# microsoft/GenerativeImage2Text

Measured on AMD Instinct MI355X. Metric: captions/sec whole-node (GIT_BASE 224px bs=64/GPU greedy len=20), higher is better.
Workload: dtype f16; 1 GPU; GIT_BASE 224px bs=64/GPU greedy max_len=20 frames=1; global_batch=64, parallelism=dp1, decode_steps_per_caption=19, seq_len_returned=20, hip_graph=True, contexts_in_flight=4, layernorm_folded=True, library=libgitmi_f16.so, encoder_chains=2, schedule=mixed

## Files before the change

generativeimage2text_amd/csrc/engine.hip:

```cpp
#include "../../include/gitmi.h"
#include "engine_state.h"

#include <algorithm>
#include <cmath>
#include <cstdarg>
#include <cstdio>
#include <cstring>

using namespace gitmi;

#ifdef GITMI_EXPERIMENT
#include "../../include/gitmi_experiment.h"
#define GITMI_EXP_EXPORT extern "C"
#else
#define GITMI_EXP_EXPORT [[maybe_unused]] static
#endif

static thread_local char g_err[1024] = "";
int gitmi::fail(const char* fmt, ...) {
    va_list ap;
    va_start(ap, fmt);
    vsnprintf(g_err, sizeof(g_err), fmt, ap);
    va_end(ap);
    return 1;
// ... 224 lines not shown
    hipDeviceSynchronize();
    if (e->enc_after) {
        auto& w = e->enc_after->enc_watchers;
        w.erase(std::remove(w.begin(), w.end(), e), w.end());
    }
    for (gitmi_engine* w : e->enc_watchers) w->enc_after = nullptr;
    destroy_graph(e);
    if (e->own_stream) hipStreamDestroy(e->own_stream);
    if (e->fence_in) hipEventDestroy(e->fence_in);
    if (e->fence_out) hipEventDestroy(e->fence_out);
    for (auto ev : e->gev)
        if (ev) hipEventDestroy(ev);
    if (e->enc_done) hipEventDestroy(e->enc_done);
    for (auto ev : e->event_pool) hipEventDestroy(ev);
    for (void* p : e->allocs) hipFree(p);
    for (void* p : e->sc_allocs) hipFree(p);
    hipFree(e->at_out); hipFree(e->at_stats); hipFree(e->ctx_tab); hipFree(e->mem_tab); hipFree(e->feat_tab); hipFree(e->ban_words);
    if (e->ban_stage) hipHostFree(e->ban_stage);
    if (e->ban_staged) hipEventDestroy(e->ban_staged);
    if (e->trie_off) hipFree(e->trie_off);
    if (e->trie_tok) hipFree(e->trie_tok);
    if (e->trie_child) hipFree(e->trie_child);
    delete e;
}

extern "C" int gitmi_set_image_shape(gitmi_engine* e, int H, int W, void* stream) {
    if (!e) return fail("null engine");
    if (!e->finalized) return fail("weights not finalized");
    const gitmi_config& c = e->cfg;
    if (H == 0 && W == 0) {
        if (!e->ragged) {
            e->ragged = true;
            e->H = e->W = e->gh = e->gw = 0;
            e->N = e->Nmax;
            drop_resident(e);
        }
        return 0;
    }
    if (H < c.patch || W < c.patch) return fail("image %dx%d is smaller than one %d-pixel patch", H, W, c.patch);
    const int gh = H / c.patch, gw = W / c.patch;
    if ((size_t)H * W > e->max_pixels)
        return fail("image %dx%d exceeds the max_image_pixels capacity (%zu)", H, W, e->max_pixels);
    if (gh * gw + 1 > e->Nmax)
        return fail("a %dx%d token grid exceeds the max_image_tokens capacity (%d)", gh, gw, e->Nmax);
    if (H == e->H && W == e->W && !e->ragged) return 0;
    e->ragged = false;
    HIPCK(hipSetDevice(e->device));
    if (gh == e->g_nat && gw == e->g_nat) {
        e->pos_cur = e->w.pos;
    } else {
        HIPCK(launch_pos_bicubic(e->w.pos, e->pos_var, e->g_nat, gh, gw, c.vit_width, (hipStream_t)stream));
        e->pos_cur = e->pos_var;
    }
    e->H = H; e->W = W; e->gh = gh; e->gw = gw; e->N = gh * gw + 1;
    drop_resident(e);
    return 0;
}

static Stream vit_stream(gitmi_engine* e, int M) {
    const int D = e->cfg.vit_width;
    const VitLayerW& L = e->w.vit[0];
    Stream st;
    st.x = e->v_x; st.M = M; st.D = D; st.tag = TAG_GEMM_VIT; st.t = e->v_h;
    st.fold = e->pol.ln_fold && on_p8(e->v_x, D, L.qkv_f.w, e->v_qkv, 3 * D, M, 3 * D, D, false) &&
              on_p8(e->v_x, D, L.ffn1_f.w, e->v_u, 4 * D, M, 4 * D, D, false) && on_p8(e->v_ctx, D, L.wo, e->v_x, D, M, D, D, true) &&
              on_p8(e->v_u, 4 * D, L.w2, e->v_x, D, M, D, 4 * D, true);
    if (st.fold) st.parts[0] = st.parts[1] = e->v_part;
    return st;
}
static Stream prefill_stream(gitmi_engine* e, int M) {
    const int d = e->cfg.dec_hidden, ffn = e->cfg.dec_ffn, D = e->cfg.vit_width;
    const DecLayerW& L = e->w.dec[0];
    Stream st;
    st.x = e->p_y; st.M = M; st.D = d; st.tag = TAG_GEMM_OTHER; st.t = e->p_ht; st.xn = e->p_hf;
    st.fold = e->pol.ln_fold && on_p8(e->feats, D, e->w.vp_w, e->p_y, d, M, d, D, true) &&
              on_p8(e->p_y, d, L.qkv_pf.w, e->img_kv[0], 3 * d, M, 3 * d, d, false) &&
              on_p8(e->p_y, d, L.qkv_pf.w, e->img_kv[0], 3 * d, M, 2 * d, d, false) &&
              (e->cfg.dec_layers < 2 || (on_p8(e->p_y, d, L.ffn1_pf.w, e->p_u, ffn, M, ffn, d, false) &&
                                         on_p8(e->p_ctx, d, L.wo, e->p_y, d, M, d, d, true) && on_p8(e->p_u, ffn, L.w2, e->p_y, d, M, d, ffn, true)));
    if (st.fold) { st.parts[0] = e->p_part[0]; st.parts[1] = e->p_part[1]; }
    return st;
}

static int encode_frames_impl(gitmi_engine* e, const float* const* frames, int F, int B, float* feats_out,
                              hipStream_t s, int stride = 0) {
    const gitmi_config& c = e->cfg;
    const int D = c.vit_width, N = e->N;
    const int F_eff = c.num_frames > 0 ? std::min(F, c.num_frames) : F;
    const int Nimg = stride > 0 ? stride : F_eff * N;
    drop_resident(e);
    SpanGuard phase(e, s, TAG_VIT, 0);
    const int BI = F_eff * B;
    const int M = BI * N;
    const int g2 = N - 1;
    const size_t slot = (size_t)3 * e->max_pixels;
    if (e->ragged)
        HIPCK(launch_im2col_ragged(e->frame_stage[0], slot, e->rg_meta, e->patches, e->pol.f32, B, N, c.patch, e->Kp, e->Kp_pad, s));
    else
    for (int fr = 0; fr < F_eff; ++fr)
        HIPCK(launch_im2col(frames[fr], (char*)e->patches + (size_t)fr * B * g2 * e->Kp_pad * e->pol.esz, e->pol.f32, B,
                            e->H, e->W, c.patch, e->Kp, e->Kp_pad, s));
    RCK(gemm(e, s, e->patches, e->Kp_pad, e->w.conv_w, nullptr, nullptr, 0, e->patch_out, D, true, BI * g2, D, e->Kp_pad, 0,
             TAG_GEMM_VIT));
    Stream x = vit_stream(e, M);
    float2* part = stream_part_out(x);
    if (e->ragged)
        HIPCK(launch_vit_assemble_ragged(e->patch_out, e->w.cls, e->w.pos, e->g_nat, e->rg_meta, e->w.lnpre_g, e->w.lnpre_b, 1e-5f, e->v_x,
                                         e->pol.stream_f16, BI, N, c.patch, D, part, s));
    else
    HIPCK(launch_vit_assemble_ln(e->patch_out, e->w.cls, e->pos_cur, e->w.lnpre_g, e->w.lnpre_b, 1e-5f, e->v_x, e->pol.stream_f16, BI, N, D,
                                 part, D / 256, s));
    stream_written(x, part, e->w.vit[0].ln1g, e->w.vit[0].ln1b, 1e-5f);
    for (int l = 0; l < c.vit_layers; ++l) {
        const VitLayerW& L = e->w.vit[l];
        const VitLayerW* Ln = l + 1 < c.vit_layers ? &e->w.vit[l + 1] : nullptr;
        RCK(ln_gemm(e, s, x, L.qkv_f, L.wqkv, L.bqkv, e->v_qkv, 3 * D, 0, 3 * D, 0));
        RCK(attn_full_packed(e, e->v_qkv, e->v_ctx, D, c.vit_heads, N, BI, e->ragged ? e->rg_ntok : nullptr, s));
        RCK(gemm_to_stream(e, s, x, e->v_ctx, D, L.wo, L.bo, D, true, L.ln2g, L.ln2b, 1e-5f));
        RCK(ln_gemm(e, s, x, L.ffn1_f, L.w1, L.b1, e->v_u, 4 * D, 0, 4 * D, 1));
        RCK(gemm_to_stream(e, s, x, e->v_u, 4 * D, L.w2, L.b2, 4 * D, true, Ln ? Ln->ln1g : nullptr, Ln ? Ln->ln1b : nullptr, 1e-5f));
    }
    for (int fr = 0; fr < F_eff; ++fr) {
        const float* te = (c.num_frames > 0 && e->pol.use_temb) ? e->w.temb[fr] : nullptr;
        if (e->pol.stream_f16) {
            const char* xs = (const char*)e->v_x + (size_t)fr * B * N * D * 2;
            HIPCK(launch_layernorm_s16(xs, D, e->w.lnpost_g, e->w.lnpost_b, 1e-5f, te, e->feats, D, false, nullptr, 0, B * N, D, N,
                                       Nimg, fr * N, s));
            if (feats_out)
                HIPCK(launch_layernorm_s16(xs, D, e->w.lnpost_g, e->w.lnpost_b, 1e-5f, te, feats_out, D, true, nullptr, 0, B * N, D,
                                           N, Nimg, fr * N, s));
        } else {
            HIPCK(launch_layernorm(e->v_x + (size_t)fr * B * N * D, D, e->w.lnpost_g, e->w.lnpost_b, 1e-5f, te, e->feats, D, e->pol.f32,
                                   feats_out, D, B * N, D, N, Nimg, fr * N, s));
        }
    }
    if (e->ragged) {
        HIPCK(launch_zero_pad_rows(e->feats, e->pol.f32, D, e->rg_ntok, B, N, s));
        if (feats_out) HIPCK(launch_zero_pad_rows(feats_out, true, D, e->rg_ntok, B, N, s));
    }

    set_resident(e, B, F_eff, stride);
    return 0;
}

static int kv_repack(gitmi_engine* e, int l, int B, int Nimg, hipStream_t s) {
    const gitmi_config& c = e->cfg;
    void* kh = e->img_kh[l];
    void* vh = e->img_vh[l];
    if (e->pol.f32) HIPCK(launch_kv_repack(e->img_kv[l], kh, vh, B, Nimg, c.dec_heads, c.dec_hidden, s));
    else HIPCK(launch_kv_repack_frag(e->img_kv[l], kh, vh, B, Nimg, round_up(Nimg, 32), c.dec_heads, c.dec_hidden, s));
    return 0;
}

static int prefill_impl(gitmi_engine* e, hipStream_t s) {
    const gitmi_config& c = e->cfg;
    const int d = c.dec_hidden, ffn = c.dec_ffn, D = c.vit_width;
    const int B = e->cur_B, Nimg = e->cur_Nimg, M = B * Nimg;
    e->have_prefill = false;
    SpanGuard phase(e, s, TAG_PREFILL, 0);
    Stream y = prefill_stream(e, M);
    RCK(gemm_to_stream(e, s, y, e->feats, D, e->w.vp_w, e->w.vp_b, D, false, e->w.vp_lng, e->w.vp_lnb, 1e-5f));
    for (int l = 0; l < c.dec_layers; ++l) {
        const DecLayerW& L = e->w.dec[l];
        const bool last = l + 1 == c.dec_layers;
        const int col0 = last ? d : 0;
        RCK(ln_gemm(e, s, y, L.qkv_pf, L.wqkv, L.bqkv, e->img_kv[l], 3 * d, col0, 3 * d - col0, 0));
        RCK(kv_repack(e, l, B, Nimg, s));
        if (last) break;
        RCK(attn_full_packed(e, e->img_kv[l], e->p_ctx, d, c.dec_heads, Nimg, B, key_counts(e), s));
        RCK(gemm_to_stream(e, s, y, e->p_ctx, d, L.wo, L.bo, d, true, L.lnag, L.lnab, 1e-12f));
        RCK(ln_gemm(e, s, y, L.ffn1_pf, L.w1, L.b1, e->p_u, ffn, 0, ffn, 2));
        RCK(gemm_to_stream(e, s, y, e->p_u, ffn, L.w2, L.b2, ffn, true, L.lnog, L.lnob, 1e-12f));
    }
    set_prefilled(e);
    return 0;
}

#ifdef GITMI_EXPERIMENT
#define GITMI_SKIPPED(e, bit) (((e)->pol.decode_skip & (bit)) != 0)
#else
#define GITMI_SKIPPED(e, bit) false
#endif
static int dgemm(gitmi_engine* e, hipStream_t s, const DGemmArgs& g_in) {
    DGemmArgs g = g_in;
    g.dbg = e->pol.dgemm_dbg;
    g.no_row_walk = e->pol.dgemm_no_row_walk >= 0 ? e->pol.dgemm_no_row_walk : e->pol.shared_device ? 0 : 1;
    g.strips_per_wg = e->pol.dgemm_strips >= 0 ? e->pol.dgemm_strips : e->pol.shared_device ? 2 : 1;
    g.rows_per_wg = e->pol.dgemm_rows > 0 ? e->pol.dgemm_rows : g.M > 64 ? 64 : e->pol.shared_device ? 32 : 16;
    SpanGuard sp(e, s, TAG_GEMM_OTHER, gemm_flops(g.M, g.N, g.K));
    HIPCK(launch_dgemm(g, s));
    return 0;
}

static DGemmArgs dgemm_ln(const void* A, const Folded& f, const DLn* ln, void* C, int c_frag, int act, int M, int N, int K) {
    return dgemm_ln(A, f.w, f.bias, f.colsum, ln, C, c_frag, act, M, N, K);
}

static int decode_layers_impl(gitmi_engine* e, const int* kv_src, int ld_ids, int pos, int R, int beams, hipStream_t s) {
    const gitmi_config& c = e->cfg;
    const int d = c.dec_hidden, ffn = c.dec_ffn;
    const int B = R / beams;
    const bool chain = e->pol.skinny && !e->pol.f32;
    for (int l = 0; l < c.dec_layers; ++l) {
        const DecLayerW& L = e->w.dec[l];
        const DecLayerW* Lp = l > 0 ? &e->w.dec[l - 1] : nullptr;
        const DLn ln_prev{e->stats_o, d / 16, 1.0f / (float)d, 1e-12f, Lp ? Lp->lnog : nullptr, Lp ? Lp->lnob : nullptr};
        const DLn ln_a{e->stats_a, d / 16, 1.0f / (float)d, 1e-12f, L.lnag, L.lnab};
        const DLn* ln_o = Lp ? &ln_prev : nullptr;
        AttnDecodeArgs a{};
        a.qkv = e->d_qkv; a.img_k = e->img_kh[l]; a.img_v = e->img_vh[l]; a.txt_k = e->txt_k[l]; a.txt_v = e->txt_v[l]; a.out = e->d_ctx;
        a.kv_src = kv_src; a.ld_src = ld_ids; a.d = d; a.N_img = e->cur_Nimg; a.T_max = c.max_text_len;
        a.img_of = e->img_identity ? nullptr : e->img_of_dev;
        a.pos = pos; a.beams = beams; a.scale = 0.125f;
        a.out_frag = chain ? 1 : 0;
        a.N_pad = round_up(e->cur_Nimg, 32);
        a.dbg = e->pol.attn_dbg;
        a.waves_per_pair = e->pol.attn_nh;
        a.pairs_per_wg = e->pol.attn_pw > 0 ? e->pol.attn_pw : e->pol.shared_device ? 8 : 4;
        const bool stream_ok = !e->pol.shared_device && a.N_pad <= 8 * 32 && B * c.dec_heads >= 384 && e->pol.attn_nh != 2;
        a.stream_wgs = e->pol.attn_stream >= 0 ? e->pol.attn_stream : stream_ok ? 192 : 0;
        if (e->keyed) { a.ntok = e->rg_ntok; a.stream_wgs = 0; }
        bool qkv_inside = false;
        if (chain) {
            const DGemmArgs g = dgemm_ln(l == 0 ? e->d_ht : e->xo_b, L.qkv_f, ln_o, e->d_qkv, 0, 0, R, 3 * d, d);
            attn_decode_set_qkv(a, g);
            qkv_inside = !GITMI_SKIPPED(e, ~0) && !e->pol.dgemm_dbg && attn_decode_qkv_form(a, B, c.dec_heads) && attn_decode_pairs_per_wg(a, B, c.dec_heads) == 8;
            if (!qkv_inside && !GITMI_SKIPPED(e, 2) && !GITMI_SKIPPED(e, 16)) RCK(dgemm(e, s, g));
        } else {
            RCK(gemm(e, s, e->d_ht, d, L.wqkv, L.bqkv, nullptr, 0, e->d_qkv, 3 * d, e->pol.f32, R, 3 * d, d, 0, TAG_GEMM_OTHER));
        }
        if (e->pol.f32) HIPCK(launch_attn_decode(a, B, c.dec_heads, s));
        else if (qkv_inside) HIPCK(launch_attn_decode_qkv(a, B, c.dec_heads, s));
        else if (!GITMI_SKIPPED(e, 1)) HIPCK(launch_attn_decode_mfma(a, B, c.dec_heads, s));
        if (chain) {
            if (!GITMI_SKIPPED(e, 4))
                RCK(dgemm(e, s, dgemm_to_stream(e->d_ctx, L.wo_p, L.bo, l == 0 ? e->d_hf : e->xo_f, ln_o, e->xa_f, e->xa_b, e->stats_a, R, d, d)));
            if (!GITMI_SKIPPED(e, 2)) RCK(dgemm(e, s, dgemm_ln(e->xa_b, L.ffn1_f, &ln_a, e->d_u, 1, 2, R, ffn, d)));
            if (!GITMI_SKIPPED(e, 4))
                RCK(dgemm(e, s, dgemm_to_stream(e->d_u, L.w2_p, L.b2, e->xa_f, &ln_a, e->xo_f, e->xo_b, e->stats_o, R, d, ffn)));
        } else {
            RCK(dec_layer_tail(e, s, L, e->d_ctx, e->d_hf, e->d_ht, e->d_y, e->d_u, R));
        }
    }
    return 0;
}

static int sample_candidates(gitmi_engine* e, const float* logits, int ldl, int R, int step, hipStream_t s, StepCands* cands,
                             const BanArgs* ban);
static int trie_candidates(gitmi_engine* e, const float* logits, int ldl, int cur_len, hipStream_t s, StepCands* cands);
static float rep_penalty_of(const gitmi_engine* e) {
    const double rp = e->sample.repetition_penalty;
    return (e->ss.kind == GITMI_SEARCH_GENERATOR && rp > 0 && rp != 1.0) ? (float)rp : 0.f;
}

static BanArgs ban_args(const gitmi_engine* e) {
    BanArgs b{};
    if (!e->ban_live || !e->ban_words) return b;
    const int mb = e->cfg.max_batch;
    b.W = (e->cfg.vocab + 31) / 32; b.eos = e->cfg.eos;
    const int* tab = reinterpret_cast<const int*>(e->ban_words + (size_t)mb * b.W);
    b.words = e->ban_words; b.set_of = tab; b.min_new = tab + mb; b.ngram = tab + 2 * mb;
    return b;
}

static int decode_head_impl(gitmi_engine* e, const int* ids, int ld_ids, int cur_len, int R, int beams, int suppress_kind,
                            int M, float* logits_out, int ldl, hipStream_t s, StepCands* cands) {
    const gitmi_config& c = e->cfg;
    const int d = c.dec_hidden;
    const bool chain = e->pol.skinny && !e->pol.f32;
    cands->part_val = e->part_val; cands->part_idx = e->part_idx; cands->part_lse = e->part_lse;
    const bool sampling = ids != nullptr && e->ss.sampled;
    const bool trie = ids != nullptr && e->trie_search;
    if ((sampling || trie) && !logits_out) { logits_out = e->logits; ldl = e->ldl; }
    const BanArgs ban = ids ? ban_args(e) : BanArgs{};
    if (chain) {
        VocabArgs v{};
        v.A = (const unsigned short*)e->xo_b; v.lda = d; v.W = (const unsigned short*)e->w.out_f.w; v.bias = e->w.out_f.bias; v.colsum = e->w.out_f.colsum;
        v.stats_in = e->stats_o; v.strips_in = d / 16; v.inv_d = 1.0f / (float)d; v.eps_in = 1e-12f;
        v.M = R; v.N = c.vocab; v.K = d; v.cols_per_wg = e->vocab_cols;
        v.max_wgs = e->pol.vocab_wgs >= 0 ? e->pol.vocab_wgs : (e->pol.shared_device && R <= 64) ? 60 : 0;
        v.ids = ids; v.ld_ids = ld_ids; v.cur_len = cur_len; v.plen = e->plen_dev; v.beams = beams; v.suppress_kind = suppress_kind;
        v.rep_penalty = ids ? rep_penalty_of(e) : 0.f;
        v.ban = ban;
        v.part_val = e->part_val; v.part_idx = e->part_idx; v.part_lse = e->part_lse;
        v.logits_out = logits_out; v.ld_logits = ldl;
        {
            SpanGuard sp(e, s, TAG_GEMM_OTHER, gemm_flops(R, c.vocab, d));
            if (!GITMI_SKIPPED(e, 8)) HIPCK(launch_vocab_topm(v, M, s));
        }
        cands->nparts = e->vocab_nparts; cands->slots = vocab_mtop_slots(M);
        if (sampling) RCK(sample_candidates(e, logits_out, ldl, R, cur_len, s, cands, nullptr));
        if (trie) RCK(trie_candidates(e, logits_out, ldl, cur_len, s, cands));
    } else {
        RCK(gemm(e, s, e->d_ht, d, e->w.out_w, e->w.out_b, nullptr, 0, e->logits, e->ldl, true, R, c.vocab, d, 0, TAG_GEMM_OTHER));
        cands->nparts = 1; cands->slots = row_topm_slots(M);
        if (sampling) RCK(sample_candidates(e, e->logits, e->ldl, R, cur_len, s, cands, &ban));
        else if (trie) RCK(trie_candidates(e, e->logits, e->ldl, cur_len, s, cands));
        else if (ids)
            HIPCK(launch_row_topm(e->logits, e->ldl, c.vocab, ids, ld_ids, cur_len, e->plen_dev, beams, suppress_kind,
                                  rep_penalty_of(e), M, R,
                                  e->part_val, e->part_idx, e->part_lse, s, &ban));
        if (logits_out && logits_out != e->logits) HIPCK(launch_copy_f32(e->logits, e->ldl, logits_out, ldl, R, c.vocab, s));
    }
    return 0;
}

static int check_ready(gitmi_engine* e) {
    if (!e) return fail("null engine");
    if (!e->finalized) return fail("weights not finalized (call gitmi_finalize_weights)");
    HIPCK(hipSetDevice(e->device));
    return 0;
}

static int ragged_prepare(gitmi_engine* e, const float* const* frames, int F, int B, hipStream_t s) {
// ... 69 lines not shown
        RCK(embed_position(e, e->ss.ids[0], T, pos, R, s));
        RCK(decode_layers_impl(e, e->ss.kv_src[0], T, pos, R, beams, s));
        if (pos == t - 1) RCK(decode_head_impl(e, nullptr, T, t, R, beams, 0, 1, logits_out, c.vocab, s, &cands));
    }
    return 0;
}

static int search_begin_impl(gitmi_engine* e, const Request& rq, int V, hipStream_t s) {
    const gitmi_config& c = e->cfg;
    const gitmi_search* sp = rq.sp;
    const int B = rq.Q, minP = rq.minP, maxP = rq.maxP;
    if (!sp) return fail("search: null config");
    if (sp->kind != GITMI_SEARCH_AUTOREGRESSIVE && sp->kind != GITMI_SEARCH_GENERATOR && sp->kind != GITMI_SEARCH_TRIE)
        return fail("search: bad kind");
    if (sp->kind == GITMI_SEARCH_TRIE) {
        if (sp->beam_size != 1) return fail("search: TrieAutoRegressiveBeamSearch asserts beam_size == 1 (trie_decoder.py:37)");
        if (!e->trie_off) return fail("search: no trie loaded (gitmi_set_trie)");
        if (sp->do_sample) return fail("search: the trie search has no sampling branch");
    }
    if (B < 1 || B > c.max_batch) return fail("search: B=%d outside [1,%d]", B, c.max_batch);
    if (sp->beam_size < 1 || sp->beam_size > c.max_beams) return fail("search: beam_size %d outside [1,%d]", sp->beam_size, c.max_beams);
    if (sp->per_node_beam_size < 1 && sp->kind != GITMI_SEARCH_TRIE) return fail("search: per_node_beam_size must be >= 1");
    if (sp->kind == GITMI_SEARCH_GENERATOR && sp->per_node_beam_size < 2)
        return fail("search: GeneratorWithBeamSearch requires per_node_beam_size > 1 (decoder.py:1078)");
    if (sp->beam_size * sp->per_node_beam_size > 16) return fail("search: beam_size*per_node_beam_size > 16 unsupported");
    if (sp->max_steps > c.max_text_len) return fail("search: max_steps %d exceeds max_text_len %d", sp->max_steps, c.max_text_len);
    if (minP < 1 || maxP > sp->max_steps) return fail("search: prefix lengths [%d,%d] outside [1,max_steps]", minP, maxP);
    if (sp->kind == GITMI_SEARCH_GENERATOR && !(sp->length_penalty > 0)) return fail("search: length_penalty must be > 0");
    if (sp->repetition_penalty != 0 && sp->repetition_penalty != 1.0) {
        if (sp->kind != GITMI_SEARCH_GENERATOR) return fail("search: repetition_penalty belongs to GeneratorWithBeamSearch (decoder.py:1064)");
        if (!(sp->repetition_penalty >= 1.0)) return fail("search: `repetition_penalty` should be >= 1 (decoder.py:1080)");
        if (sp->max_steps > 1024) return fail("search: repetition_penalty supports histories up to 1024 tokens");
    }
    if (sp->num_keep_best < 0 || sp->num_keep_best > SS_NHMAX) return fail("search: num_keep_best %d outside [1,%d]", sp->num_keep_best, SS_NHMAX);
    if (sp->num_keep_best > 1 && sp->kind != GITMI_SEARCH_GENERATOR)
        return fail("search: num_keep_best belongs to GeneratorWithBeamSearch.search (decoder.py:1087)");
    if (sp->do_sample) {
        if (sp->kind != GITMI_SEARCH_GENERATOR) return fail("search: do_sample is implemented for GeneratorWithBeamSearch (decoder.py:1146-1166) only");
        if (sp->temperature < 0) return fail("search: temperature must be > 0");
        if (V > 32768) return fail("search: sampling supports vocabularies up to 32768 tokens");
    }
    SearchState& st = e->ss;
    e->trie_search = sp->kind == GITMI_SEARCH_TRIE;
    st.B = B; st.k = sp->beam_size; st.pn = e->trie_search ? 1 : sp->per_node_beam_size;
    st.T = sp->max_steps;
    st.V = V; st.eos = c.eos; st.kind = e->trie_search ? GITMI_SEARCH_AUTOREGRESSIVE : sp->kind; st.length_penalty = sp->length_penalty;
    st.prefixed = rq.prefixed ? 1 : 0;
    st.nh = keep_best(*sp);
    st.sampled = sp->do_sample ? 1 : 0;
    e->sample = *sp;
    st.start = e->start_dev; st.ld_start = c.max_text_len; st.plen = e->plen_dev;
    e->ss_cur = 0; e->ss_len = minP;
    HIPCK(launch_search_init(st, s));
    if (e->trie_search) HIPCK(launch_fill_i32(e->trie_cursor, 0, B, s));
    return 0;
}

static int search_mtop(const SearchState& st) {
    if (st.sampled) return st.pn;
    return st.kind == GITMI_SEARCH_AUTOREGRESSIVE ? std::max(st.k, st.pn) : st.pn * st.k;
}
static int sample_candidates(gitmi_engine* e, const float* logits, int ldl, int R, int step, hipStream_t s, StepCands* cands,
                             const BanArgs* ban) {
    const gitmi_search& sp = e->sample;
    const float temp = sp.temperature > 0 ? (float)sp.temperature : 1.0f;
    HIPCK(launch_sample_rows(logits, ldl, e->ss.V, R, temp, sp.top_k, (float)sp.top_p, e->ss.pn, sp.seed, step,
                             e->part_val, e->part_idx, e->part_lse, nullptr, e->ss.ids[e->ss_cur], e->ss.T, step,
                             rep_penalty_of(e), row_topm_slots(e->ss.pn), s, ban, e->plen_dev, e->ss.k));
    cands->part_val = e->part_val; cands->part_idx = e->part_idx; cands->part_lse = e->part_lse;
    cands->nparts = 1; cands->slots = row_topm_slots(e->ss.pn);
    return 0;
}

static int trie_candidates(gitmi_engine* e, const float* logits, int ldl, int cur_len, hipStream_t s, StepCands* cands) {
    const SearchState& st = e->ss;
    TrieArgs tr{e->trie_off, e->trie_tok, e->trie_child, e->trie_cursor};
    HIPCK(launch_trie_select(logits, ldl, st.V, st.ids[e->ss_cur], st.T, cur_len, e->plen_dev, st.eos, tr, st.B, e->part_val,
                             e->part_idx, e->part_lse, s));
    cands->part_val = e->part_val; cands->part_idx = e->part_idx; cands->part_lse = e->part_lse;
    cands->nparts = 1; cands->slots = 1;
    return 0;
}

static int search_step_impl(gitmi_engine* e, const StepCands& cands, bool embed, hipStream_t s) {
    const SearchState& st = e->ss;
    const int cur_len = e->ss_len;
    if (cur_len >= st.T) return fail("search_advance: sequence already at max_steps");
    HIPCK(launch_search_step(st, e->ss_cur, cur_len, cands, embed_args(e, embed), e->pol.f32, s));
    e->ss_cur ^= 1;
    e->ss_len = cur_len + 1;
    return 0;
}

static int fill_uniform_sentences(gitmi_engine* e, int B, const long long* prefix_dev, int P, hipStream_t s) {
    HIPCK(launch_fill_start(e->start_dev, e->cfg.max_text_len, prefix_dev, 0, 1, e->cfg.sos, B, P, s));
    HIPCK(launch_fill_i32(e->plen_dev, P, B, s));
    e->img_identity = true;
    return 0;
}

extern "C" int gitmi_set_trie(gitmi_engine* e, int n_nodes, const int32_t* child_off, const int32_t* child_tok,
                              const int32_t* child_node) {
    RCK(check_ready(e));
    HIPCK(hipDeviceSynchronize());
    destroy_graph(e);
    int *n_off = nullptr, *n_tok = nullptr, *n_child = nullptr;
    if (n_nodes > 0) {
        if (!child_off || child_off[0] != 0) return fail("set_trie: child_off must start at 0");
        const int n_edges = child_off[n_nodes];
        for (int n = 0; n < n_nodes; ++n)
            if (child_off[n + 1] < child_off[n]) return fail("set_trie: child_off must be non-decreasing");
        if (n_edges > 0 && (!child_tok || !child_node)) return fail("set_trie: null edge arrays");
        for (int i = 0; i < n_edges; ++i)
            if (child_node[i] < 0 || child_node[i] >= n_nodes) return fail("set_trie: edge %d leads to node %d of %d", i, child_node[i], n_nodes);
        hipError_t err = hipMalloc((void**)&n_off, (size_t)(n_nodes + 1) * sizeof(int));
        if (err == hipSuccess) err = hipMalloc((void**)&n_tok, (size_t)std::max(n_edges, 1) * sizeof(int));
        if (err == hipSuccess) err = hipMalloc((void**)&n_child, (size_t)std::max(n_edges, 1) * sizeof(int));
        if (err == hipSuccess) err = hipMemcpy(n_off, child_off, (size_t)(n_nodes + 1) * sizeof(int), hipMemcpyHostToDevice);
        if (err == hipSuccess && n_edges > 0) err = hipMemcpy(n_tok, child_tok, (size_t)n_edges * sizeof(int), hipMemcpyHostToDevice);
        if (err == hipSuccess && n_edges > 0) err = hipMemcpy(n_child, child_node, (size_t)n_edges * sizeof(int), hipMemcpyHostToDevice);
        if (err != hipSuccess) {
            if (n_off) hipFree(n_off);
            if (n_tok) hipFree(n_tok);
            if (n_child) hipFree(n_child);
            return fail("set_trie: %s (the previous trie is kept)", hipGetErrorString(err));
        }
    }
    if (e->trie_off) { hipFree(e->trie_off); hipFree(e->trie_tok); hipFree(e->trie_child); }
    e->trie_off = n_off; e->trie_tok = n_tok; e->trie_child = n_child;
    return 0;
}

static int search_begin_host(gitmi_engine* e, const char* who, const gitmi_search* sp, int B, const int64_t* start_host, int ld,
                             const int32_t* plen_host, int vocab, void* stream) {
    RCK(check_ready(e));
    if (!start_host) return fail("%s: null start", who);
    if (B < 1 || B > e->cfg.max_batch || ld < 1 || ld > e->cfg.max_text_len) return fail("%s: bad B/P", who);
    if (vocab < 2) return fail("%s: bad vocab", who);
    if (sp && sp->kind == GITMI_SEARCH_SCORE) return fail("%s: GITMI_SEARCH_SCORE is not a search (gitmi_generate_prefixed scores sentences)", who);
    if (sp && sp->kind == GITMI_SEARCH_ATTEND) return fail("%s: GITMI_SEARCH_ATTEND is not a search (gitmi_generate_prefixed returns the attention maps of sentences)", who);
    if (sp && sp->kind == GITMI_SEARCH_CONTEXT) return fail("%s: GITMI_SEARCH_CONTEXT is not a search (gitmi_generate_prefixed puts context tokens into the decoder memory)", who);
    if (sp && sp->kind == GITMI_SEARCH_TREE_SCORE) return fail("%s: GITMI_SEARCH_TREE_SCORE is not a search (gitmi_generate_prefixed scores token trees)", who);
    if (sp && sp->kind == GITMI_SEARCH_KEEP) return fail("%s: GITMI_SEARCH_KEEP is not a search (gitmi_generate_prefixed keeps the memory of resident images)", who);
    if (sp && sp->kind == GITMI_SEARCH_RECALL) return fail("%s: GITMI_SEARCH_RECALL is not a search (gitmi_generate_prefixed recalls kept images)", who);
    if (sp && sp->kind == GITMI_SEARCH_FEATURES) return fail("%s: GITMI_SEARCH_FEATURES is not a search (gitmi_generate_prefixed installs given feature rows)", who);
    if (sp && sp->kind == GITMI_SEARCH_CONSTRAIN) return fail("%s: GITMI_SEARCH_CONSTRAIN is not a search (gitmi_generate_prefixed arms the constraints of the next search call)", who);
    if (e->ban_armed)
        return fail("%s: decoding constraints are armed for %d sentences (GITMI_SEARCH_CONSTRAIN): the seam's caller owns its logits and "
                    "applies its own -- disarm first (a GITMI_SEARCH_CONSTRAIN call with Q == 0)", who, e->ban_armed);
    e->ban_live = false;
    int minP = ld, maxP = ld;
    if (plen_host) {
        maxP = 1;
        for (int b = 0; b < B; ++b) {
            if (plen_host[b] < 1 || plen_host[b] > ld) return fail("%s: prefix length %d of sentence %d outside [1,%d]", who, plen_host[b], b, ld);
            minP = std::min(minP, (int)plen_host[b]); maxP = std::max(maxP, (int)plen_host[b]);
        }
    }
    hipStream_t s = (hipStream_t)stream;
    HIPCK(hipMemcpy2DAsync(e->start_dev, (size_t)e->cfg.max_text_len * sizeof(long long), start_host,
                           (size_t)ld * sizeof(long long), (size_t)ld * sizeof(long long), (size_t)B, hipMemcpyHostToDevice, s));
    if (plen_host) HIPCK(hipMemcpyAsync(e->plen_dev, plen_host, (size_t)B * sizeof(int), hipMemcpyHostToDevice, s));
    HIPCK(hipStreamSynchronize(s));
    if (!plen_host) HIPCK(launch_fill_i32(e->plen_dev, ld, B, s));
    e->img_identity = true;
    Request rq{};
    rq.Q = B; rq.minP = minP; rq.maxP = maxP; rq.prefixed = plen_host != nullptr; rq.sp = sp;
    return search_begin_impl(e, rq, vocab, s);
}

extern "C" int gitmi_search_begin(gitmi_engine* e, const gitmi_search* sp, int B, const int64_t* start_host, int P,
// ... 1 lines not shown
    return search_begin_host(e, "search_begin", sp, B, start_host, P, nullptr, vocab, stream);
}

extern "C" int gitmi_search_rows(gitmi_engine* e, int64_t* tokens_out, int* R, int* t, void* stream) {
    RCK(check_ready(e));
    const SearchState& st = e->ss;
    if (R) *R = st.B * st.k;
    if (t) *t = e->ss_len;
    if (tokens_out) HIPCK(launch_search_rows(st, e->ss_cur, e->ss_len, (long long*)tokens_out, (hipStream_t)stream));
    return 0;
}

extern "C" int gitmi_search_advance(gitmi_engine* e, const float* logits, void* stream) {
    RCK(check_ready(e));
    if (!logits) return fail("search_advance: null logits");
    const SearchState& st = e->ss;
    hipStream_t s = (hipStream_t)stream;
    const int M = search_mtop(st), R = st.B * st.k;
    StepCands cands{e->part_val, e->part_idx, e->part_lse, 1, row_topm_slots(M)};
    if (st.sampled) RCK(sample_candidates(e, logits, st.V, R, e->ss_len, s, &cands, nullptr));
    else if (e->trie_search) RCK(trie_candidates(e, logits, st.V, e->ss_len, s, &cands));
    else
        HIPCK(launch_row_topm(logits, st.V, st.V, st.ids[e->ss_cur], st.T, e->ss_len, e->plen_dev, st.k,
                              st.kind == GITMI_SEARCH_AUTOREGRESSIVE ? 1 : 0, rep_penalty_of(e), M, R, e->part_val,
                              e->part_idx, e->part_lse, s));
    return search_step_impl(e, cands, false, s);
}

extern "C" int gitmi_search_done_count(gitmi_engine* e, int* done_out, void* stream) {
    RCK(check_ready(e));
    if (!done_out) return fail("search_done_count: null argument");
    int h = 0;
    HIPCK(hipMemcpyAsync(&h, e->ss.info, sizeof(int), hipMemcpyDeviceToHost, (hipStream_t)stream));
    HIPCK(hipStreamSynchronize((hipStream_t)stream));
    *done_out = h;
    return 0;
}

extern "C" int gitmi_search_finish(gitmi_engine* e, int64_t* tokens_out, float* logprob_out, int32_t* info_out,
                                   void* stream) {
    RCK(check_ready(e));
    const SearchState& st = e->ss;
    HIPCK(launch_search_finish(st, e->ss_cur, e->ss_len, (long long*)tokens_out, logprob_out, info_out, nullptr,
                               (hipStream_t)stream));
    return 0;
}

GITMI_EXP_EXPORT int gitmi_debug_search_begin_prefixed(gitmi_engine* e, const gitmi_search* sp, int B, const int64_t* start_host,
                                                       int ld, const int32_t* plen_host, int vocab, void* stream) {
    if (!plen_host) return fail("debug_search_begin_prefixed: null prefix lengths");
    return search_begin_host(e, "debug_search_begin_prefixed", sp, B, start_host, ld, plen_host, vocab, stream);
}
GITMI_EXP_EXPORT int gitmi_debug_search_advance_lists(gitmi_engine* e, const float* part_val, const int* part_idx,
                                                      const float* part_lse, int nparts, int slots, int embed, void* stream) {
    RCK(check_ready(e));
    if (!part_val || !part_idx || !part_lse) return fail("debug_search_advance_lists: null argument");
    const SearchState& st = e->ss;
    if (st.B < 1 || st.T < 1) return fail("debug_search_advance_lists: no search has begun");
    if (st.sampled || e->trie_search) return fail("debug_search_advance_lists: the sampling and trie searches select from whole logit rows");
    if (nparts < 1 || nparts > 256) return fail("debug_search_advance_lists: nparts=%d outside [1,256]", nparts);
    if (slots != 1 && slots != 2 && slots != 4 && slots != 8 && slots != 16)
        return fail("debug_search_advance_lists: slots=%d is not one of 1, 2, 4, 8, 16", slots);
    if (slots < search_mtop(st)) return fail("debug_search_advance_lists: slots=%d, but the step reads %d candidates per row", slots, search_mtop(st));
    const StepCands cands{part_val, part_idx, (const float2*)part_lse, nparts, slots};
    return search_step_impl(e, cands, embed != 0, (hipStream_t)stream);
}
GITMI_EXP_EXPORT int gitmi_debug_read_hidden(gitmi_engine* e, int R, float* hf_out, void* ht_out, int* ht_frag, int* ht_dtype,
                                             void* stream) {
    RCK(check_ready(e));
    const gitmi_config& c = e->cfg;
    if (R < 1 || R > c.max_batch * c.max_beams) return fail("debug_read_hidden: R=%d outside the capacity", R);
    if (!hf_out || !ht_out || !ht_frag || !ht_dtype) return fail("debug_read_hidden: null argument");
    hipStream_t s = (hipStream_t)stream;
    const size_t D = (size_t)c.dec_hidden, Rp = (size_t)(R + 15) / 16 * 16;
    HIPCK(hipMemcpyAsync(hf_out, e->d_hf, (size_t)R * D * sizeof(float), hipMemcpyDefault, s));
    HIPCK(hipMemcpyAsync(ht_out, e->d_ht, Rp * D * e->pol.esz, hipMemcpyDefault, s));
    HIPCK(hipStreamSynchronize(s));
    *ht_frag = (e->pol.skinny && !e->pol.f32) ? 1 : 0;
    *ht_dtype = e->pol.f32 ? GITMI_DTYPE_F32 : gitmi_operand_dtype();
    return 0;
}

static int generate_encode(gitmi_engine* e, const Request& rq, hipStream_t s) {
    RCK(encode_frames_impl(e, rq.frames, rq.F, rq.B, nullptr, s));
    return prefill_impl(e, s);
}
static int images_ready(gitmi_engine* e, const Request& rq, hipStream_t s) {
    if (rq.frames) return generate_encode(e, rq, s);
    return e->have_prefill ? 0 : prefill_impl(e, s);
}

static int generate_decode(gitmi_engine* e, const Request& rq, hipStream_t s, bool allow_poll) {
    const gitmi_config& c = e->cfg;
    const gitmi_search* sp = rq.sp;
    RCK(search_begin_impl(e, rq, c.vocab, s));
    const int Q = rq.Q, minP = rq.minP, maxP = rq.maxP, T = sp->max_steps, k = sp->beam_size, R = Q * k;
    const SearchState& st = e->ss;
    const int M = search_mtop(st);
    const int suppress = sp->kind != GITMI_SEARCH_GENERATOR ? 1 : 0;
    {
        SpanGuard phase(e, s, TAG_DECODE, 0);
        RCK(embed_position(e, st.ids[0], T, 0, R, s));
        e->ss_len = 1;
        StepCands cands{e->part_val, e->part_idx, e->part_lse, 1, 1};
        while (e->ss_len < T) {
            const int cur_len = e->ss_len;
            SpanGuard step(e, s, TAG_STEP, 0);
            RCK(decode_layers_impl(e, st.kv_src[e->ss_cur], T, cur_len - 1, R, k, s));
            if (cur_len >= minP)
                RCK(decode_head_impl(e, st.ids[e->ss_cur], T, cur_len, R, k, suppress, M, nullptr, 0, s, &cands));
            RCK(search_step_impl(e, cands, true, s));
            if (allow_poll && e->ss_len > maxP && (e->ss_len - maxP) % 8 == 0 && e->ss_len < T) {
                int h[4];
                HIPCK(hipMemcpyAsync(h, st.info, sizeof(h), hipMemcpyDeviceToHost, s));
                HIPCK(hipStreamSynchronize(s));
                if (h[0] >= Q) break;
            }
        }
    }
    HIPCK(launch_search_finish(st, e->ss_cur, e->ss_len, rq.tokens, rq.logprob, rq.info, rq.sent, s));
    if (e->ragged)
        HIPCK(launch_ragged_report(e->rg_meta, e->img_identity ? nullptr : e->img_of_dev, Q, keep_best(*sp), rq.logprob, rq.info,
                                   nullptr, s));
    const double kv = (double)Q * c.dec_layers * 2.0 * ((double)e->cur_Nimg + k * 0.5 * (minP + T)) * c.dec_hidden * e->pol.esz;
    e->last_decode_step_bytes = e->w.dec_weight_bytes + kv;
    return 0;
}

static int generate_body(gitmi_engine* e, const Request& rq, hipStream_t s, bool allow_poll) {
    SpanGuard total(e, s, 99, 0);
    RCK(images_ready(e, rq, s));
    return generate_decode(e, rq, s, allow_poll);
}

static GraphKey graph_key_of(const gitmi_engine* e, const Request& rq, int F_eff) {
    const gitmi_search& sp = *rq.sp;
    const bool resident = rq.frames == nullptr;
    return {rq.B, rq.Q, F_eff, rq.minP, sp.kind, sp.beam_size, sp.per_node_beam_size, sp.max_steps, e->H, e->W,
            rq.prefixed ? 1 : 0, e->img_identity ? 1 : 0, e->pol.use_temb ? 1 : 0, resident ? 1 : 0,
            resident ? e->cur_Nimg : 0, resident && e->keyed ? 1 : 0, sp.length_penalty,
            sp.do_sample, sp.top_k, keep_best(sp), sp.top_p, sp.temperature, sp.repetition_penalty, sp.seed, e->ban_live ? 1 : 0};
}

static int replay(gitmi_engine* e, const Request& rq, hipStream_t x, const CapturedGraph* enc, const CapturedGraph* dec) {
    const bool timed = e->profile_mode == 2;
    if (timed) {
        for (auto& ev : e->gev)
            if (!ev) HIPCK(hipEventCreate(&ev));
        HIPCK(hipEventRecord(e->gev[enc ? 0 : 1], x));
    } else if (enc && e->enc_after && e->enc_after->enc_done) {
        HIPCK(hipStreamWaitEvent(x, e->enc_after->enc_done, 0));
    }
    if (enc) {
        HIPCK(enc->launch(x));
        if (timed) HIPCK(hipEventRecord(e->gev[1], x));
        else if (e->enc_done && !e->enc_watchers.empty()) HIPCK(hipEventRecord(e->enc_done, x));
    }
    if (dec) HIPCK(dec->launch(x));
    if (!timed) return 0;
    HIPCK(hipEventRecord(e->gev[2], x));
    HIPCK(hipStreamSynchronize(x));
    float a = 0, b = 0;
    if (enc) HIPCK(hipEventElapsedTime(&a, e->gev[0], e->gev[1]));
    HIPCK(hipEventElapsedTime(&b, e->gev[1], e->gev[2]));
    e->split_encode_ms += a; e->split_decode_ms += b; e->split_calls += 1; e->split_steps += rq.sp->max_steps - 1;
    return 0;
}

static int generate_graphed(gitmi_engine* e, const Request& rq, hipStream_t s) {
    const gitmi_config& c = e->cfg;
    const bool resident = rq.frames == nullptr;
    hipStream_t x = s ? s : e->own_stream;
    if (x != s) {
        HIPCK(hipEventRecord(e->fence_in, s));
        HIPCK(hipStreamWaitEvent(x, e->fence_in, 0));
    }
    const size_t frame_bytes = (size_t)rq.B * 3 * e->H * e->W * sizeof(float);
    const int F_eff = resident ? e->cur_F : c.num_frames > 0 ? std::min(rq.F, c.num_frames) : rq.F;
    if (!e->ragged && !resident)
    for (int f = 0; f < F_eff; ++f)
        HIPCK(hipMemcpyAsync(e->frame_stage[f], rq.frames[f], frame_bytes, hipMemcpyDeviceToDevice, x));
    Request own = rq;
    if (!resident) { own.frames = e->frame_stage.data(); own.F = F_eff; }
    own.tokens = e->out_tokens; own.logprob = e->out_lp; own.info = e->out_info; own.sent = e->out_sent;
    const GraphKey key = graph_key_of(e, rq, F_eff);
    const CapturedGraph *enc = nullptr, *dec = nullptr;
    if (resident) {
        RCK(images_ready(e, rq, x));
        if (!e->follow_slot.valid || !(key == e->follow_slot.key)) {
            e->follow_slot.valid = false;
            RCK(e->graph_follow.capture(x, [&] { return generate_decode(e, own, x, false); }));
            e->follow_slot = {key, true};
        }
        dec = &e->graph_follow;
    } else {
        const bool split = e->profile_mode == 2 || e->enc_after != nullptr || !e->enc_watchers.empty();
        if (!e->full_slot.valid || !(key == e->full_slot.key) || split != e->graph_is_split) {
            e->full_slot.valid = false;
            e->graph_decode.reset();
            if (!split) {
                RCK(e->graph_full.capture(x, [&] { return generate_body(e, own, x, false); }));
            } else {
                RCK(e->graph_full.capture(x, [&] { return generate_encode(e, own, x); }));
                RCK(e->graph_decode.capture(x, [&] { return generate_decode(e, own, x, false); }));
            }
            e->full_slot = {key, true}; e->graph_is_split = split;
        } else {
            set_resident(e, rq.B, F_eff);
            set_prefilled(e);
        }
        enc = &e->graph_full;
        if (split) dec = &e->graph_decode;
    }
    RCK(replay(e, rq, x, enc, dec));
    const size_t nout = (size_t)rq.Q * (size_t)keep_best(*rq.sp);
    HIPCK(hipMemcpyAsync(rq.tokens, e->out_tokens, nout * rq.sp->max_steps * sizeof(long long), hipMemcpyDefault, x));
    HIPCK(hipMemcpyAsync(rq.logprob, e->out_lp, nout * sizeof(float), hipMemcpyDefault, x));
    HIPCK(hipMemcpyAsync(rq.info, e->out_info, 4 * sizeof(int), hipMemcpyDefault, x));
    if (rq.sent != e->out_sent) HIPCK(hipMemcpyAsync(rq.sent, e->out_sent, (size_t)rq.Q * 2 * sizeof(int), hipMemcpyDefault, x));
    if (x != s) {
        HIPCK(hipEventRecord(e->fence_out, x));
        HIPCK(hipStreamWaitEvent(s, e->fence_out, 0));
    }
    return 0;
}

static int generate_run(gitmi_engine* e, const Request& rq, hipStream_t s, bool constrained) {
    const bool long_budget = rq.sp->max_steps - rq.minP > 32;
    const bool graph = e->pol.use_graph && !e->profiling && !long_budget;
    if (constrained) e->ban_armed = 0;
    e->ban_live = constrained;
    const int rc = settle_residency(e, rq, graph ? generate_graphed(e, rq, s) : generate_body(e, rq, s, long_budget && !e->profiling));
    e->ban_live = false;
    return rc;
}

static int constrain_check(const gitmi_engine* e, const char* who, const gitmi_search* sp, int Q, bool* constrained);

extern "C" int gitmi_generate(gitmi_engine* e, const float* const* frames, int F, int B, const int64_t* prefix, int P,
                              const gitmi_search* sp, int64_t* tokens_out, float* logprob_out, int32_t* info_out,
                              void* stream) {
    RCK(check_ready(e));
    const gitmi_config& c = e->cfg;
    if (sp && sp->kind == GITMI_SEARCH_SCORE) return fail("generate: GITMI_SEARCH_SCORE scores given sentences: call gitmi_generate_prefixed");
    if (sp && sp->kind == GITMI_SEARCH_ATTEND) return fail("generate: GITMI_SEARCH_ATTEND maps given sentences: call gitmi_generate_prefixed");
    if (sp && sp->kind == GITMI_SEARCH_CONTEXT) return fail("generate: GITMI_SEARCH_CONTEXT takes context segments: call gitmi_generate_prefixed");
    if (sp && sp->kind == GITMI_SEARCH_TREE_SCORE) return fail("generate: GITMI_SEARCH_TREE_SCORE scores given token trees: call gitmi_generate_prefixed");
    if (sp && sp->kind == GITMI_SEARCH_KEEP) return fail("generate: GITMI_SEARCH_KEEP keeps the memory of resident images: call gitmi_generate_prefixed");
    if (sp && sp->kind == GITMI_SEARCH_RECALL) return fail("generate: GITMI_SEARCH_RECALL recalls kept images: call gitmi_generate_prefixed");
    if (sp && sp->kind == GITMI_SEARCH_FEATURES) return fail("generate: GITMI_SEARCH_FEATURES installs given feature rows: call gitmi_generate_prefixed");
    if (sp && sp->kind == GITMI_SEARCH_CONSTRAIN) return fail("generate: GITMI_SEARCH_CONSTRAIN arms decoding constraints: call gitmi_generate_prefixed");
    if (!frames) RCK(check_resident(e, "generate", B));
    if (!sp || !tokens_out || !logprob_out || !info_out) return fail("generate: null argument");
    if (frames) RCK(check_frames(e, "generate", frames, F, B));
    if (!prefix) P = 1;
    if (P < 1 || P > c.max_text_len) return fail("generate: prefix length %d outside [1,%d]", P, c.max_text_len);
    if (sp->max_steps < P || sp->max_steps > c.max_text_len) return fail("generate: max_steps %d outside [P,%d]", sp->max_steps, c.max_text_len);
    bool constrained = false;
    RCK(constrain_check(e, "generate", sp, B, &constrained));
    hipStream_t s = (hipStream_t)stream;
    if (frames) RCK(ragged_prepare(e, frames, F, B, s));
    RCK(fill_uniform_sentences(e, B, (const long long*)prefix, P, s));
    const Request rq{frames, F, B, B, P, P, false, sp, (long long*)tokens_out, logprob_out, info_out, e->out_sent};
    return generate_run(e, rq, s, constrained);
}

static int tree_max_depth(const gitmi_config& c) { return std::min((int)c.max_text_len, (int)c.max_pos); }
constexpr int TREE_MAX_ROWS = 65535 * 64;
static void score_free(gitmi_engine* e) {
    for (void* p : e->sc_allocs) hipFree(p);
    e->sc_allocs.clear();
    e->sc_rows = 0;
    e->tr_out_n = 0;
}
static int score_alloc(gitmi_engine* e, size_t rows_needed, size_t tree_out = 0) {
    size_t rows = (size_t)round_up((int)rows_needed, 128);
    if (e->sc_rows >= rows && e->tr_out_n >= tree_out) return 0;
    rows = std::max(rows, e->sc_rows);
    tree_out = std::max(tree_out, e->tr_out_n);
    score_free(e);
    const gitmi_config& c = e->cfg;
    const int d = c.dec_hidden;
    const size_t Qmax = (size_t)c.max_batch * c.max_beams;
    const size_t esz = e->pol.esz;
    auto alloc = [&](auto** p, size_t bytes) -> bool {
        void* q = nullptr;
        if (hipMalloc(&q, bytes) != hipSuccess) return false;
        e->sc_allocs.push_back(q);
        *reinterpret_cast<void**>(p) = q;
        return true;
    };
    const bool ok = alloc(&e->sc_hf, rows * d * 4) && alloc(&e->sc_y, rows * d * 4) && alloc(&e->sc_ht, rows * d * esz) &&
                    alloc(&e->sc_qkv, rows * 3 * d * esz) && alloc(&e->sc_ctx, rows * d * esz) &&
                    alloc(&e->sc_u, rows * c.dec_ffn * esz) &&
                    alloc(&e->sc_part, rows * (size_t)(e->pol.f32 ? 1 : score_head_tiles(c.vocab)) * sizeof(float4)) &&
                    alloc(&e->sc_zt, rows * 4) && alloc(&e->sc_tgt, rows * 4) && alloc(&e->sc_lens, Qmax * 4) &&
                    alloc(&e->sc_img, Qmax * 4) && alloc(&e->sc_bad, Qmax * 4) && alloc(&e->sc_info, 16) &&
// ... 722 lines not shown
```

generativeimage2text_amd/csrc/engine_state.h:

```cpp
#pragma once
#include "../../include/gitmi.h"
#include "abi_common.h"
#include "launchers.h"

#include <hip/hip_runtime.h>

#include <functional>
#include <map>
#include <string>
#include <tuple>
#include <vector>

static inline int round_up(int x, int m) { return (x + m - 1) / m * m; }
static inline int keep_best(const gitmi_search& sp) { return sp.num_keep_best > 1 ? sp.num_keep_best : 1; }

struct HostTensor {
    std::vector<float> data;
    std::vector<int64_t> shape;
    float amax = 0.f;
    size_t numel() const { size_t n = 1; for (auto s : shape) n *= (size_t)s; return n; }
};

struct Folded { void* w = nullptr; float* bias = nullptr; float* colsum = nullptr; };

struct VitLayerW {
    void *wqkv = nullptr, *wo = nullptr, *w1 = nullptr, *w2 = nullptr;
    float *bqkv = nullptr, *bo = nullptr, *b1 = nullptr, *b2 = nullptr;
    float *ln1g = nullptr, *ln1b = nullptr, *ln2g = nullptr, *ln2b = nullptr;
    Folded qkv_f;
    Folded ffn1_f;
};
struct DecLayerW {
    void *wqkv = nullptr, *wo = nullptr, *w1 = nullptr, *w2 = nullptr;
    float *bqkv = nullptr, *bo = nullptr, *b1 = nullptr, *b2 = nullptr;
    float *lnag = nullptr, *lnab = nullptr, *lnog = nullptr, *lnob = nullptr;
    Folded qkv_f;
    Folded ffn1_f;
    void *wo_p = nullptr, *w2_p = nullptr;
    Folded qkv_pf, ffn1_pf;
};

struct TimedSpan { hipEvent_t a, b; int tag; double flops; };
enum { TAG_VIT = 0, TAG_PREFILL = 1, TAG_DECODE = 2, TAG_GEMM_VIT = 10, TAG_GEMM_OTHER = 11, TAG_STEP = 20 };

struct GraphKey {
    int B, Q, F, P, kind, k, pn, T, H, W, prefixed, ident, temb, resident, Nimg, keyed; double lp;
    int smp, top_k, nh; double top_p, temp, rp; unsigned long long seed;
    int constrained;
    auto fields() const {
        return std::tie(B, Q, F, P, kind, k, pn, T, H, W, prefixed, ident, temb, resident, Nimg, keyed, lp, smp, top_k, nh, top_p, temp,
                        rp, seed, constrained);
    }
    bool operator==(const GraphKey& o) const { return fields() == o.fields(); }
};
struct GraphSlot { GraphKey key{}; bool valid = false; };

struct CapturedGraph {
    hipGraph_t graph = nullptr;
    hipGraphExec_t exec = nullptr;
    void reset() {
        if (exec) hipGraphExecDestroy(exec);
        if (graph) hipGraphDestroy(graph);
        exec = nullptr, graph = nullptr;
    }
    int capture(hipStream_t s, const std::function<int()>& fn);
    hipError_t launch(hipStream_t s) const { return hipGraphLaunch(exec, s); }
};

struct Request {
    const float* const* frames;
    int F, B, Q, minP, maxP;
    bool prefixed;
    const gitmi_search* sp;
    long long* tokens; float* logprob; int32_t* info;
    int32_t* sent;
};

struct ModelWeights {
    void* conv_w = nullptr;
    float *cls = nullptr, *pos = nullptr, *lnpre_g = nullptr, *lnpre_b = nullptr, *lnpost_g = nullptr, *lnpost_b = nullptr;
    std::vector<VitLayerW> vit;
    std::vector<float*> temb;
    void* vp_w = nullptr;
    float *vp_b = nullptr, *vp_lng = nullptr, *vp_lnb = nullptr;
    float *words_f = nullptr, *positions_f = nullptr, *emb_lng = nullptr, *emb_lnb = nullptr;
    std::vector<DecLayerW> dec;
    void* out_w = nullptr;
    float* out_b = nullptr;
    Folded out_f;
    double dec_weight_bytes = 0;
};

struct Policy {
    bool f32 = false;
    size_t esz = 2;
    int attn_impl = 1;
    bool stream_f16 = false;
    bool ln_fold = false;
    bool ln_fold_ready = false;
    bool skinny = true;
    bool use_graph = true;
    bool use_temb = true;
    bool shared_device = false;
    int attn_dbg = 0, dgemm_dbg = 0;
    int attn_pw = 0;
    int attn_nh = 0;
    int attn_stream = -1;
    int dgemm_no_row_walk = -1;
    int dgemm_strips = -1;
    int vocab_wgs = -1;
    int gemm_tall = 1;
    int dgemm_rows = 0;
    int decode_skip = 0;
};

struct gitmi_engine {
    gitmi_config cfg{};
    ModelWeights w;
    Policy pol;
    int device = 0;
    bool finalized = false;
    gitmi_engine* parent = nullptr;

    std::map<std::string, HostTensor> host_w;
    std::vector<void*> allocs;

    int N = 0, gh = 0, gw = 0, H = 0, W = 0, Kp = 0, Kp_pad = 0;
    int N_nat = 0, g_nat = 0, Nmax = 0;
    size_t max_pixels = 0;
    float* pos_var = nullptr;
    const float* pos_cur = nullptr;
    bool ragged = false;
    int4* rg_meta = nullptr;
    int* rg_ntok = nullptr;
    bool keyed = false;
    bool has_context = false;
    int* ctx_tab = nullptr;
    size_t ctx_tab_ints = 0;
    gitmi::MemoryEntry* mem_tab = nullptr;
    size_t mem_tab_n = 0;
    std::vector<int4> res_desc;
    gitmi::FeaturePiece* feat_tab = nullptr;
    unsigned int* ban_words = nullptr;
    int* ban_stage = nullptr;
    hipEvent_t ban_staged = nullptr;
    int ban_armed = 0;
    bool ban_live = false;

    void *patches = nullptr, *v_h = nullptr, *v_qkv = nullptr, *v_ctx = nullptr, *v_u = nullptr;
    float *patch_out = nullptr, *v_x = nullptr;
    void* feats = nullptr;
    float *p_y = nullptr, *p_hf = nullptr;
    void *p_ht = nullptr, *p_ctx = nullptr, *p_u = nullptr;
    std::vector<void*> img_kv;
    std::vector<void*> img_kh, img_vh;
    float *d_y = nullptr, *d_hf = nullptr, *logits = nullptr;
    void *d_ht = nullptr, *d_qkv = nullptr, *d_ctx = nullptr, *d_u = nullptr;
    std::vector<void*> txt_k, txt_v;
// ... 63 lines not shown
```

generativeimage2text_amd/csrc/engine_weights.hip:

```cpp
#include "engine_state.h"

#include <algorithm>
#include <cmath>
#include <cstring>

using namespace gitmi;

static int dev_alloc(gitmi_engine* e, void** p, size_t bytes) {
    if (bytes == 0) bytes = 16;
    HIPCK(hipMalloc(p, bytes));
    e->allocs.push_back(*p);
    return 0;
}
template <typename T> static int dev_alloc_t(gitmi_engine* e, T** p, size_t count) {
    return dev_alloc(e, reinterpret_cast<void**>(p), count * sizeof(T));
}

static float half_to_float(uint16_t h) {
    const uint32_t sign = (uint32_t)(h & 0x8000) << 16;
    uint32_t exp = (h >> 10) & 0x1f, man = h & 0x3ff, out;
    if (exp == 0) {
        if (man == 0) out = sign;
        else {
            exp = 127 - 15 + 1;
// ... 103 lines not shown
    RCK(dev_alloc(e, &e->patches, (size_t)c.max_batch * c.max_frames * (e->Nmax - 1) * e->Kp_pad * esz));
    RCK(dev_alloc_t(e, &e->patch_out, (size_t)c.max_batch * c.max_frames * (e->Nmax - 1) * D));
    RCK(dev_alloc_t(e, &e->pos_var, (size_t)e->Nmax * D));
    RCK(dev_alloc_t(e, &e->v_x, Mv * D));
    RCK(dev_alloc(e, &e->v_h, Mv * D * esz));
    RCK(dev_alloc(e, &e->v_qkv, Mv * 3 * D * esz));
    RCK(dev_alloc(e, &e->v_ctx, Mv * D * esz));
    RCK(dev_alloc(e, &e->v_u, Mv * 4 * D * esz));
    RCK(dev_alloc(e, &e->feats, Mp * D * esz));
    if (e->pol.ln_fold_ready) {
        RCK(dev_alloc_t(e, &e->v_part, Mv * 4));
        RCK(dev_alloc_t(e, &e->p_part[0], Mp * 4));
        RCK(dev_alloc_t(e, &e->p_part[1], Mp * 4));
        HIPCK(hipMemset(e->v_part, 0, Mv * 4 * sizeof(float2)));
        HIPCK(hipMemset(e->p_part[0], 0, Mp * 4 * sizeof(float2)));
        HIPCK(hipMemset(e->p_part[1], 0, Mp * 4 * sizeof(float2)));
    }
    RCK(dev_alloc_t(e, &e->p_y, Mp * d));
    RCK(dev_alloc_t(e, &e->p_hf, Mp * d));
    RCK(dev_alloc(e, &e->p_ht, Mp * d * esz));
    RCK(dev_alloc(e, &e->p_ctx, Mp * d * esz));
    RCK(dev_alloc(e, &e->p_u, Mp * c.dec_ffn * esz));
    e->img_kv.resize(c.dec_layers);
    e->img_kh.resize(c.dec_layers);
    e->img_vh.resize(c.dec_layers);
    e->txt_k.resize(c.dec_layers);
    e->txt_v.resize(c.dec_layers);
    for (int l = 0; l < c.dec_layers; ++l) {
        RCK(dev_alloc(e, &e->img_kv[l], Mp * 3 * d * esz));
        const size_t Mkv = (size_t)c.max_batch * round_up(c.max_frames * e->Nmax, 32);
        RCK(dev_alloc(e, &e->img_kh[l], Mkv * d * esz));
        RCK(dev_alloc(e, &e->img_vh[l], Mkv * d * esz));
        RCK(dev_alloc(e, &e->txt_k[l], R * T * d * esz));
        RCK(dev_alloc(e, &e->txt_v[l], R * T * d * esz));
    }
    RCK(dev_alloc_t(e, &e->d_y, R * d));
    RCK(dev_alloc_t(e, &e->d_hf, R * d));
    RCK(dev_alloc(e, &e->d_ht, R * d * esz));
    RCK(dev_alloc(e, &e->d_qkv, R * 3 * d * esz));
    RCK(dev_alloc(e, &e->d_ctx, R * d * esz));
    RCK(dev_alloc(e, &e->d_u, R * c.dec_ffn * esz));
    RCK(dev_alloc_t(e, &e->xa_f, R * d));
    RCK(dev_alloc_t(e, &e->xo_f, R * d));
    RCK(dev_alloc(e, &e->xa_b, R * d * 2));
    RCK(dev_alloc(e, &e->xo_b, R * d * 2));
    RCK(dev_alloc_t(e, &e->stats_a, R * (size_t)(d / 16)));
    RCK(dev_alloc_t(e, &e->stats_o, R * (size_t)(d / 16)));
    e->ldl = round_up(c.vocab, 8);
    RCK(dev_alloc_t(e, &e->logits, R * e->ldl));
    e->vocab_cols = 128;
    e->vocab_nparts = (e->pol.skinny && !e->pol.f32) ? vocab_parts(c.vocab, e->vocab_cols) : 1;
    RCK(dev_alloc_t(e, &e->part_val, R * (size_t)e->vocab_nparts * 16));
    RCK(dev_alloc_t(e, &e->part_idx, R * (size_t)e->vocab_nparts * 16));
    RCK(dev_alloc_t(e, &e->part_lse, R * (size_t)e->vocab_nparts));
    SearchState& s = e->ss;
    for (int i = 0; i < 2; ++i) {
        RCK(dev_alloc_t(e, &s.ids[i], R * T));
        RCK(dev_alloc_t(e, &s.kv_src[i], R * T));
        RCK(dev_alloc_t(e, &s.score[i], R));
    }
    RCK(dev_alloc_t(e, &s.done, (size_t)c.max_batch));
    RCK(dev_alloc_t(e, &s.hyp_n, (size_t)c.max_batch));
    RCK(dev_alloc_t(e, &s.hyp_cnt, (size_t)c.max_batch));
    RCK(dev_alloc_t(e, &s.hyp_worst, (size_t)c.max_batch));
    RCK(dev_alloc_t(e, &s.hyp_score, (size_t)c.max_batch * SS_NHMAX));
    RCK(dev_alloc_t(e, &s.hyp_len, (size_t)c.max_batch * SS_NHMAX));
    RCK(dev_alloc_t(e, &s.hyp_seq, (size_t)c.max_batch * SS_NHMAX));
    RCK(dev_alloc_t(e, &s.hyp_tok, (size_t)c.max_batch * SS_NHMAX * T));
    RCK(dev_alloc_t(e, &s.stop, (size_t)c.max_batch));
    RCK(dev_alloc_t(e, &s.early, (size_t)c.max_batch));
    RCK(dev_alloc_t(e, &s.info, 4));
    RCK(dev_alloc_t(e, &s.len_norm, (size_t)T + 1));
    RCK(dev_alloc_t(e, &e->start_dev, (size_t)c.max_batch * T));
    RCK(dev_alloc_t(e, &e->plen_dev, (size_t)c.max_batch));
    RCK(dev_alloc_t(e, &e->img_of_dev, (size_t)c.max_batch));
    RCK(dev_alloc_t(e, &e->trie_cursor, (size_t)c.max_batch));
    RCK(dev_alloc_t(e, &e->out_tokens, (size_t)c.max_batch * SS_NHMAX * T));
    RCK(dev_alloc_t(e, &e->out_lp, (size_t)c.max_batch * SS_NHMAX));
    RCK(dev_alloc_t(e, &e->out_info, 4));
    RCK(dev_alloc_t(e, &e->out_sent, (size_t)c.max_batch * 2));
    HIPCK(hipStreamCreateWithFlags(&e->own_stream, hipStreamNonBlocking));
    HIPCK(hipEventCreateWithFlags(&e->fence_in, hipEventDisableTiming));
    HIPCK(hipEventCreateWithFlags(&e->fence_out, hipEventDisableTiming));
    e->frame_stage.resize(c.max_frames);
    for (int f = 0; f < c.max_frames; ++f)
        RCK(dev_alloc_t(e, &e->frame_stage[f], (size_t)c.max_batch * 3 * e->max_pixels));
    RCK(dev_alloc_t(e, &e->rg_meta, (size_t)c.max_batch));
    RCK(dev_alloc_t(e, &e->rg_ntok, (size_t)c.max_batch));
    return 0;
}

#ifdef GITMI_OPS_F16
static inline float bf16_round(float f) { return (float)(_Float16)f; }
#else
static inline float bf16_round(float f) {
    uint32_t u;
    memcpy(&u, &f, 4);
    if ((u & 0x7f800000u) == 0x7f800000u) return f;
    u += 0x7fffu + ((u >> 16) & 1u);
    u &= 0xffff0000u;
    memcpy(&f, &u, 4);
    return f;
}
#endif
static int fold_layernorm(gitmi_engine* e, const std::vector<float>& W, const std::vector<float>& bias,
                          const std::vector<float>& gamma, const std::vector<float>& beta, int64_t rows, int K, bool frag,
                          Folded* out) {
    std::vector<float> wf((size_t)rows * K), b2((size_t)rows), c2((size_t)rows);
    float amax = 0.f;
    for (int64_t n = 0; n < rows; ++n) {
        double sum = 0.0, cst = bias[n];
        const float* w = &W[(size_t)n * K];
        float* o = &wf[(size_t)n * K];
        for (int k = 0; k < K; ++k) {
            amax = std::max(amax, std::fabs(w[k] * gamma[k]));
            o[k] = bf16_round(w[k] * gamma[k]);
            sum += (double)o[k];
            cst += (double)beta[k] * (double)w[k];
        }
        c2[n] = (float)sum;
        b2[n] = (float)cst;
    }
    RCK(operand_range_check(e, "a matrix with the LayerNorm gain in front of it folded in (W . gamma)", amax));
    const int64_t rows_pad = (rows + 127) / 128 * 128;
    RCK(dev_alloc(e, &out->w, (size_t)rows_pad * K * 2));
    float* tmp = nullptr;
    void* tmp_b = nullptr;
    HIPCK(hipMalloc((void**)&tmp, wf.size() * 4));
    hipError_t err = hipSuccess;
    if (frag) err = hipMalloc(&tmp_b, wf.size() * 2);
    if (err == hipSuccess) err = hipMemcpy(tmp, wf.data(), wf.size() * 4, hipMemcpyHostToDevice);
    if (err == hipSuccess) err = launch_convert_pad(tmp, frag ? tmp_b : out->w, false, (size_t)rows, K, K, 0);
    if (err == hipSuccess && frag) err = launch_frag_pack(tmp_b, out->w, (int)rows, (int)rows_pad, K, 0);
    if (err == hipSuccess) err = hipDeviceSynchronize();
    hipFree(tmp);
    if (tmp_b) hipFree(tmp_b);
    HIPCK(err);
    b2.resize((size_t)rows_pad, 0.f);
    c2.resize((size_t)rows_pad, 0.f);
    RCK(dev_alloc_t(e, &out->bias, (size_t)rows_pad));
    RCK(dev_alloc_t(e, &out->colsum, (size_t)rows_pad));
    HIPCK(hipMemcpy(out->bias, b2.data(), (size_t)rows_pad * 4, hipMemcpyHostToDevice));
    HIPCK(hipMemcpy(out->colsum, c2.data(), (size_t)rows_pad * 4, hipMemcpyHostToDevice));
    return 0;
}
static int pack_frag(gitmi_engine* e, const void* src, int64_t rows, int K, void** dst) {
    const int64_t rows_pad = (rows + 15) / 16 * 16;
    RCK(dev_alloc(e, dst, (size_t)rows_pad * K * 2));
    HIPCK(launch_frag_pack(src, *dst, (int)rows, (int)rows_pad, K, 0));
    HIPCK(hipDeviceSynchronize());
    return 0;
}
static int fold_named(gitmi_engine* e, const std::string& ln, const std::string& dense, int64_t rows, int K, bool frag, Folded* out) {
    const HostTensor *g, *b, *w, *bi;
    RCK(get_w(e, ln + "weight", {K}, &g));
    RCK(get_w(e, ln + "bias", {K}, &b));
    RCK(get_w(e, dense + "weight", {rows, K}, &w));
    RCK(get_w(e, dense + "bias", {rows}, &bi));
    return fold_layernorm(e, w->data, bi->data, g->data, b->data, rows, K, frag, out);
}
static std::string vit_layer_key(int i) { return "image_encoder.transformer.resblocks." + std::to_string(i) + "."; }
static std::string dec_layer_key(int i) { return "textual.transformer.encoder.layer." + std::to_string(i) + "."; }
static int concat_qkv(gitmi_engine* e, const std::string& pre, int d) {
    HostTensor w, b;
    w.shape = {3 * d, d};
    b.shape = {3 * d};
    for (const char* name : {"query", "key", "value"}) {
        const HostTensor *tw, *tb;
        RCK(get_w(e, pre + "attention.self." + name + ".weight", {d, d}, &tw));
// ... 151 lines not shown
```

generativeimage2text_amd/csrc/kernels_attn_decode.hip:

```cpp
#include "gitmi_common.h"
#include "launchers.h"
#include "dgemm_shared.h"
#include <algorithm>
#include <type_traits>

#pragma clang fp contract(off)

namespace gitmi {

static constexpr int HD = 64;

__global__ __launch_bounds__(256) void kv_repack_frag_kernel(const bf16_t* __restrict__ qkv, bf16_t* __restrict__ kf,
                                                             bf16_t* __restrict__ vt, int N, int Np, int H, int d) {
    __shared__ bf16_t vs[32][HD + 8];
    const int s = blockIdx.x, h = blockIdx.y, b = blockIdx.z, tid = threadIdx.x;
    const int nsteps = Np >> 5;
    bf16_t* kdst = kf + ((size_t)b * H + h) * Np * HD;
    bf16_t* vdst = vt + ((size_t)b * H + h) * Np * HD;
    const int key = tid >> 3, ch = tid & 7;
    const int n = s * 32 + key;
    u32x4_t kv = {0u, 0u, 0u, 0u}, vv = kv;
    if (n < N) {
        const bf16_t* src = qkv + ((size_t)b * N + n) * 3 * d + d + h * HD + ch * 8;
        kv = *reinterpret_cast<const u32x4_t*>(src);
        vv = *reinterpret_cast<const u32x4_t*>(src + d);
    }
    *reinterpret_cast<u32x4_t*>(kdst + frag_tile(n >> 4, ch >> 2, 2, (ch & 3) * 16 + (n & 15))) = kv;
    *reinterpret_cast<u32x4_t*>(&vs[key][ch * 8]) = vv;
    __syncthreads();
    const int dt = tid >> 6, lane = tid & 63, lg = lane >> 4, dim = dt * 16 + (lane & 15);
    bf16_t o[8];
#pragma unroll
    for (int e = 0; e < 8; ++e) o[e] = vs[(e >> 2) * 16 + lg * 4 + (e & 3)][dim];
    u32x4_t ov;
#pragma unroll
    for (int e = 0; e < 4; ++e) ov[e] = (uint32_t)o[2 * e] | ((uint32_t)o[2 * e + 1] << 16);
    *reinterpret_cast<u32x4_t*>(vdst + (((size_t)s * 4 + dt) * 64 + lane) * 8) = ov;
}

__device__ __forceinline__ void unpack8(const u32x4_t& r, float (&v)[8]) {
#pragma unroll
    for (int i = 0; i < 4; ++i) {
        unpack2op(r[i], v[2 * i], v[2 * i + 1]);
    }
}
__device__ __forceinline__ void ld8bf(const bf16_t* p, float (&v)[8]) { unpack8(*reinterpret_cast<const u32x4_t*>(p), v); }

constexpr int ACS = 4;

struct Pair {
    int h, row0;
    bool on;
};

struct QkvSrc {
    const bf16_t* q0;
    int row_stride, part;
    __device__ __forceinline__ const bf16_t* q(int j) const { return q0 + (size_t)j * row_stride; }
    __device__ __forceinline__ const bf16_t* k(int j) const { return q(j) + part; }
    __device__ __forceinline__ const bf16_t* v(int j) const { return q(j) + 2 * part; }
};
__device__ __forceinline__ QkvSrc qkv_rows(const AttnDecodeArgs& a, const Pair& p) {
    return QkvSrc{reinterpret_cast<const bf16_t*>(a.qkv) + (size_t)p.row0 * (3 * a.d) + p.h * HD, 3 * a.d, a.d};
}

template <int KB>
__device__ __forceinline__ void load_text_kv(const AttnDecodeArgs& a, const Pair& p, const QkvSrc& qs, int j, int s, int sub, u32x4_t& kr, u32x4_t& vr) {
    if (s == a.pos) {
        kr = *reinterpret_cast<const u32x4_t*>(qs.k(j) + sub * 8);
        vr = *reinterpret_cast<const u32x4_t*>(qs.v(j) + sub * 8);
    } else {
        const int srow = KB == 1 ? p.row0 : a.kv_src[(size_t)(p.row0 + j) * a.ld_src + s];
        const size_t off = ((size_t)srow * a.T_max + s) * a.d + p.h * HD + sub * 8;
        kr = *reinterpret_cast<const u32x4_t*>(reinterpret_cast<const bf16_t*>(a.txt_k) + off);
        vr = *reinterpret_cast<const u32x4_t*>(reinterpret_cast<const bf16_t*>(a.txt_v) + off);
    }
}

template <int KB, int TI>
struct TextItems {
    int j[TI];
    u32x4_t kr[TI], vr[TI];
    __device__ __forceinline__ void load(const AttnDecodeArgs& a, const Pair& p, const QkvSrc& qs, int grp, int ngrp, int sub) {
        const int nt = a.pos + 1;
#pragma unroll
// ... 242 lines not shown
    auto load_chunk = [&](int s0) {
#pragma unroll
        for (int c = 0; c < ACS; ++c) {
            const int s = s0 + NH * c;
            const bool on = s < nimg_steps && !(a.dbg & 8);
            const bf16_t* kp = Kf + frag_tile(2 * s, 0, 2, lane);
            const bf16_t* vp = Vt + ((size_t)s * 4 * 64 + lane) * 8;
#pragma unroll
            for (int t = 0; t < 2; ++t)
#pragma unroll
                for (int ds = 0; ds < 2; ++ds) {
                    const bf16x8_t* q = reinterpret_cast<const bf16x8_t*>(kp + (t * 2 + ds) * 512);
                    kq[c][t][ds] = !on ? bf16x8_t{0, 0, 0, 0, 0, 0, 0, 0} : (a.dbg & 16) ? *q : __builtin_nontemporal_load(q);
                }
#pragma unroll
            for (int dt = 0; dt < 4; ++dt) {
                const bf16x8_t* q = reinterpret_cast<const bf16x8_t*>(vp + dt * 512);
                vq[c][dt] = !on ? bf16x8_t{0, 0, 0, 0, 0, 0, 0, 0} : (a.dbg & 16) ? *q : __builtin_nontemporal_load(q);
            }
        }
    };
    load_chunk(half);

    const int t = tid % PT, grp = t >> 3, sub = tid & 7;
    const QkvSrc qs = qkv_rows(a, p);
    TextItems<KB, TI> ti;
    ti.load(a, p, qs, grp, 8 * NH, sub);
    append_text_cache(a, p, qs, t, sub);
    bf16x8_t qf[2];
    load_q_frag(a, p, qs, l15, lg, qf);

    ImagePartial ip;
    ip.init();
    for (int s0 = half; s0 < nimg_steps; s0 += NH * ACS) {
        if (s0 != half) load_chunk(s0);
        f32x4_t sc[ACS][2];
        float cm = -INFINITY;
#pragma unroll
        for (int c = 0; c < ACS; ++c) {
#pragma unroll
            for (int u = 0; u < 2; ++u) {
                sc[c][u] = mfma16(kq[c][u][0], qf[0], f32x4_t{0.f, 0.f, 0.f, 0.f});
                sc[c][u] = mfma16(kq[c][u][1], qf[1], sc[c][u]);
            }
            ip.mask_max(sc[c], s0 + NH * c, nimg_steps, RAGGED ? n_img : a.N_img, lg, cm);
        }
        const float mn = ip.new_max(cm, s0 != half);
#pragma unroll
        for (int c = 0; c < ACS; ++c) {
            const bf16x8_t pf = ip.p_frag(sc[c], mn);
            if (a.dbg & 4) {
#pragma unroll
                for (int dt = 0; dt < 4; ++dt) asm volatile("" ::"v"(vq[c][dt]));
                asm volatile("" ::"v"(pf));
                continue;
            }
#pragma unroll
            for (int dt = 0; dt < 4; ++dt) ip.o[dt] = mfma16(vq[c][dt], pf, ip.o[dt]);
        }
    }
    ip.finish();
    TextPartial<KB> tp;
    tp.init(a, p, qs, sub);
    tp.items(ti, !(a.dbg & 2));
    tp.template tail<TI>(a, p, qs, grp, 8 * NH, sub);
    tp.merge_groups();
    ip.publish(part[hp][half], k, l15, lg);
    if constexpr (NH > 1) __syncthreads(); else __builtin_amdgcn_wave_barrier();
    tp.fold_into(part[hp][half], k, lane, sub);
    if constexpr (NH > 1) __syncthreads(); else __builtin_amdgcn_wave_barrier();
    if constexpr (NH == 1) write_rows(a, p, part[hp][0], t, PT);
    else write_rows(a, p, part[hp][0], part[hp][NH - 1], t, PT);
}

constexpr int AQ_PW = 8;
constexpr int AQ_STRIPS = 3 * HD / 16;

__device__ __forceinline__ void attn_lds_barrier() {
    asm volatile("s_waitcnt lgkmcnt(0)" ::: "memory");
    __builtin_amdgcn_s_barrier();
    asm volatile("" ::: "memory");
}

template <int TI>
__global__ __launch_bounds__(64 * AQ_PW) void attn_decode_qkv_kernel(AttnDecodeArgs a) {
    constexpr int KB = 1;
    __shared__ __attribute__((aligned(16))) f32x4_t red[AQ_STRIPS][4][1][64];
    __shared__ __attribute__((aligned(16))) bf16_t rows[AQ_PW][3 * HD];
    __shared__ float part[AQ_PW][KB][HD + 2];

    const int tid = threadIdx.x, lane = tid & 63;
    const int wave = __builtin_amdgcn_readfirstlane(tid >> 6);
    const int l15 = lane & 15, lg = lane >> 4;
    const int H = a.d / HD, B = a.n_pairs / H;
    const int Np = a.N_pad, nsteps = Np >> 5;
    const int nsb = (B + AQ_PW - 1) / AQ_PW, total = H * nsb, per = (total + 7) >> 3;
    const int blk = (int)(blockIdx.x & 7) * per + (int)(blockIdx.x >> 3);
    if (blk >= total) return;
    const int b0 = (blk % nsb) * AQ_PW;
    Pair p;
    p.h = blk / nsb;
    p.on = b0 + wave < B;
    const int b = p.on ? b0 + wave : 0;
    p.row0 = b;
    const int bi = a.img_of ? a.img_of[b] : b;
    const bf16_t* Kf = reinterpret_cast<const bf16_t*>(a.img_k) + ((size_t)bi * H + p.h) * Np * HD;
    const bf16_t* Vt = reinterpret_cast<const bf16_t*>(a.img_v) + ((size_t)bi * H + p.h) * Np * HD;
    const int nimg_steps = p.on ? nsteps : 0;

    bf16x8_t kq[ACS][2][2], vq[ACS][4];
    auto load_k = [&](int s0) {
#pragma unroll
        for (int c = 0; c < ACS; ++c) {
            const bool on = s0 + c < nimg_steps;
            const bf16_t* kp = Kf + frag_tile(2 * (s0 + c), 0, 2, lane);
#pragma unroll
            for (int t = 0; t < 2; ++t)
#pragma unroll
                for (int ds = 0; ds < 2; ++ds)
                    kq[c][t][ds] = !on ? bf16x8_t{0, 0, 0, 0, 0, 0, 0, 0}
                                       : __builtin_nontemporal_load(reinterpret_cast<const bf16x8_t*>(kp + (t * 2 + ds) * 512));
        }
    };
    auto load_v = [&](int s0) {
#pragma unroll
        for (int c = 0; c < ACS; ++c) {
            const bool on = s0 + c < nimg_steps;
            const bf16_t* vp = Vt + ((size_t)(s0 + c) * 4 * 64 + lane) * 8;
#pragma unroll
            for (int dt = 0; dt < 4; ++dt)
                vq[c][dt] = !on ? bf16x8_t{0, 0, 0, 0, 0, 0, 0, 0}
                                : __builtin_nontemporal_load(reinterpret_cast<const bf16x8_t*>(vp + dt * 512));
        }
    };
    load_k(0);

    const int ksteps = a.d >> 5, N = 3 * a.d;
    const int slice = wave & 3;
    const KSlice ks = k_slice(ksteps, 4, slice);
    const int rt = b0 >> 4;
    auto strip_of = [&](int ls) { return (ls >> 2) * (a.d >> 4) + p.h * 4 + (ls & 3); };
    bf16x8_t xf[DW_KS][1];
    load_x_slice(xf, reinterpret_cast<const bf16_t*>(a.x), rt, ks, ksteps, lane);
#pragma unroll 2
    for (int u = 0; u < AQ_STRIPS / 2; ++u) {
        const int ls = (wave >> 2) * (AQ_STRIPS / 2) + u;
        const WSlice wf = load_w_slice<false>(reinterpret_cast<const bf16_t*>(a.w), strip_of(ls), ks, ksteps, lane);
        f32x4_t acc[1] = {f32x4_t{0.f, 0.f, 0.f, 0.f}};
        mfma_slice(acc, wf, xf, ks);
        red[ls][slice][0][lane] = acc[0];
    }
    load_v(0);
    const int fm_raw = rt * 16 + l15;
    const int fm = fm_raw < a.M ? fm_raw : a.M - 1;
    const bool second = wave + AQ_PW < AQ_STRIPS;
    const int fn0 = strip_of(wave) * 16 + lg * 4, fn1 = strip_of(second ? wave + AQ_PW : wave) * 16 + lg * 4;
    RowStatLoads sl;
    if (a.stats_in) stats_issue(sl, a.stats_in, a.strips_in, a.M, fm, lg);
    const float4 bias4[2] = {load_cols4(a.bias, fn0, N), load_cols4(a.bias, fn1, N)};
    float4 cs4[2] = {float4{0.f, 0.f, 0.f, 0.f}, float4{0.f, 0.f, 0.f, 0.f}};
    if (a.stats_in) { cs4[0] = load_cols4(a.colsum, fn0, N); cs4[1] = load_cols4(a.colsum, fn1, N); }
    attn_lds_barrier();
    {
#pragma clang fp contract(fast)
        float mean = 0.f, rstd = 1.f;
        if (a.stats_in) stats_finish(sl, a.inv_d, a.eps_in, mean, rstd);
        const int i = l15 - (b0 & 15);
#pragma unroll
        for (int t = 0; t < 2; ++t) {
            if (t == 1 && !second) break;
            const int ls = wave + t * AQ_PW;
            const f32x4_t tot = sum_waves<4>(red[ls], 0, lane);
            DGEMM_CONSUMER_FINISH(v, tot, bias4[t], cs4[t], a.stats_in, mean, rstd, GITMI_ACT_NONE);
            if (i >= 0 && i < AQ_PW) {
                uint2 o;
                o.x = pack2bf(v[0], v[1]);
                o.y = pack2bf(v[2], v[3]);
                *reinterpret_cast<uint2*>(&rows[i][ls * 16 + lg * 4]) = o;
            }
        }
    }
    attn_lds_barrier();
    const QkvSrc qs{rows[wave], 0, HD};

    const int grp = lane >> 3, sub = lane & 7;
    TextItems<KB, TI> ti;
    ti.load(a, p, qs, grp, 8, sub);
    append_text_cache(a, p, qs, lane, sub);
    bf16x8_t qf[2];
    load_q_frag(a, p, qs, l15, lg, qf);

    ImagePartial ip;
    ip.init();
    for (int s0 = 0; s0 < nimg_steps; s0 += ACS) {
        if (s0 != 0) { load_k(s0); load_v(s0); }
        f32x4_t sc[ACS][2];
        float cm = -INFINITY;
#pragma unroll
        for (int c = 0; c < ACS; ++c) {
#pragma unroll
            for (int u = 0; u < 2; ++u) {
                sc[c][u] = mfma16(kq[c][u][0], qf[0], f32x4_t{0.f, 0.f, 0.f, 0.f});
                sc[c][u] = mfma16(kq[c][u][1], qf[1], sc[c][u]);
            }
            ip.mask_max(sc[c], s0 + c, nimg_steps, a.N_img, lg, cm);
        }
        const float mn = ip.new_max(cm, s0 != 0);
#pragma unroll
        for (int c = 0; c < ACS; ++c) {
            const bf16x8_t pf = ip.p_frag(sc[c], mn);
#pragma unroll
            for (int dt = 0; dt < 4; ++dt) ip.o[dt] = mfma16(vq[c][dt], pf, ip.o[dt]);
        }
    }
    ip.finish();
    TextPartial<KB> tp;
    tp.init(a, p, qs, sub);
    tp.items(ti, true);
    tp.template tail<TI>(a, p, qs, grp, 8, sub);
    tp.merge_groups();
    ip.publish(part[wave], a.beams, l15, lg);
    __builtin_amdgcn_wave_barrier();
    tp.fold_into(part[wave], a.beams, lane, sub);
    __builtin_amdgcn_wave_barrier();
    write_rows(a, p, part[wave], lane, 64);
}
// ... 115 lines not shown
                    __builtin_amdgcn_sched_barrier(0);
#pragma unroll
                    for (int t = 0; t < 2; ++t) {
                        sc[c][t] = mfma16(kq[t][0], qf[0], f32x4_t{0.f, 0.f, 0.f, 0.f});
                        sc[c][t] = mfma16(kq[t][1], qf[1], sc[c][t]);
                    }
                    slot_done();
                } else {
                    sc[c][0] = f32x4_t{0.f, 0.f, 0.f, 0.f};
                    sc[c][1] = sc[c][0];
                }
                ip.mask_max(sc[c], s0 + c, nsteps, a.N_img, lg, cm);
            }
            const float mn = ip.new_max(cm, s0 != 0);
#pragma unroll
            for (int c = 0; c < ACS; ++c) {
                const bf16x8_t pf = ip.p_frag(sc[c], mn);
                if (s0 + c < nsteps) {
                    const unsigned char* sl = slot_ready();
                    bf16x8_t vq[4];
#pragma unroll
                    for (int dt = 0; dt < 4; ++dt) vq[dt] = *reinterpret_cast<const bf16x8_t*>(sl + dt * 1024 + lane * 16);
                    __builtin_amdgcn_sched_barrier(0);
#pragma unroll
                    for (int dt = 0; dt < 4; ++dt) ip.o[dt] = mfma16(vq[dt], pf, ip.o[dt]);
                    slot_done();
                } else {
#pragma unroll
                    for (int dt = 0; dt < 4; ++dt) ip.o[dt] = mfma16(bf16x8_t{0, 0, 0, 0, 0, 0, 0, 0}, pf, ip.o[dt]);
                }
            }
        }
        ip.finish();
        TextPartial<KB> tp;
        tp.init(a, p, qs, sub);
        tp.items(ti, true);
        tp.template tail<TI>(a, p, qs, grp, 8, sub);
        tp.merge_groups();
        ip.publish(part[wave], k, l15, lg);
        __builtin_amdgcn_wave_barrier();
        tp.fold_into(part[wave], k, lane, sub);
        __builtin_amdgcn_wave_barrier();
        write_rows(a, p, part[wave], lane, 64);
        __builtin_amdgcn_wave_barrier();
    }
}

hipError_t launch_kv_repack_frag(const void* qkv, void* kf, void* vt, int B, int N, int N_pad, int H, int d, hipStream_t s) {
    if (B <= 0 || N <= 0) return hipSuccess;
    if (N_pad % 32 || N_pad < N) return hipErrorInvalidValue;
    hipLaunchKernelGGL(kv_repack_frag_kernel, dim3(N_pad / 32, H, B), dim3(256), 0, s, (const bf16_t*)qkv, (bf16_t*)kf,
                       (bf16_t*)vt, N, N_pad, H, d);
    return hipGetLastError();
}

template <typename F>
static void with_beam_rows(int beams, F&& f) {
    if (beams <= 1) f(std::integral_constant<int, 1>{});
    else if (beams <= 2) f(std::integral_constant<int, 2>{});
    else if (beams <= 4) f(std::integral_constant<int, 4>{});
    else f(std::integral_constant<int, 8>{});
}

int attn_decode_pairs_per_wg(const AttnDecodeArgs& a, int B, int H) {
    int pw = a.pairs_per_wg >= 8 ? 8 : a.pairs_per_wg >= 4 || a.pairs_per_wg <= 0 ? 4 : a.pairs_per_wg >= 2 ? 2 : 1;
    while (pw > 1 && B * H / pw < 96) pw >>= 1;
    if (a.beams > 4 && pw == 8) pw = 4;
    return pw;
}

bool attn_decode_qkv_form(const AttnDecodeArgs& a, int B, int H) {
    if (B <= 0 || a.beams != 1 || a.waves_per_pair == 2 || a.ntok || a.stream_wgs != 0 || a.dbg) return false;
    if (a.N_img < 1 || a.N_pad % 32 || a.N_pad < a.N_img || a.N_pad > 8 * 32) return false;
    if (a.d != H * HD || a.d > 4 * DW_KS * 32 || a.M < B) return false;
    if (!a.x || !a.w || !a.bias) return false;
    return !a.stats_in || (a.colsum && a.strips_in >= 1 && a.strips_in <= 4 * STRIP_SLOTS);
}

hipError_t launch_attn_decode_qkv(const AttnDecodeArgs& a, int B, int H, hipStream_t s) {
    if (!attn_decode_qkv_form(a, B, H)) return hipErrorInvalidValue;
    AttnDecodeArgs p = a;
    p.n_pairs = B * H;
    const int total = H * ((B + AQ_PW - 1) / AQ_PW);
    hipLaunchKernelGGL((attn_decode_qkv_kernel<3>), dim3(8 * ((total + 7) / 8)), dim3(64 * AQ_PW), 0, s, p);
    return hipGetLastError();
}

hipError_t launch_attn_decode_mfma(const AttnDecodeArgs& a, int B, int H, hipStream_t s) {
    if (B <= 0) return hipSuccess;
    if (a.beams > 8 || a.N_pad % 32 || a.N_pad < a.N_img || a.N_img < 1) return hipErrorInvalidValue;
    if (a.ntok && a.stream_wgs > 0) return hipErrorInvalidValue;
    AttnDecodeArgs p = a;
    p.n_pairs = B * H;
    if (a.stream_wgs > 0) {
        const int nwg = std::max(1, std::min(a.stream_wgs, (p.n_pairs + AS_WAVES - 1) / AS_WAVES));
        with_beam_rows(a.beams, [&](auto kb) {
            constexpr int KB = decltype(kb)::value;
            hipLaunchKernelGGL((attn_decode_stream_kernel<KB, 3, KB == 8 ? 8 : 9>), dim3(nwg), dim3(64 * AS_WAVES), 0, s, p);
        });
        return hipGetLastError();
    }
    const bool one_wave = a.waves_per_pair == 1 || (a.waves_per_pair != 2 && a.N_pad <= 8 * 32);
    if (a.ntok || !one_wave) {
        with_beam_rows(a.beams, [&](auto kb) {
            constexpr int KB = decltype(kb)::value;
            if (a.ntok) hipLaunchKernelGGL((attn_decode_mfma_kernel<KB, 3, 1, 2, true>), dim3(H, B), dim3(128), 0, s, p);
            else hipLaunchKernelGGL((attn_decode_mfma_kernel<KB>), dim3(H, B), dim3(128), 0, s, p);
        });
        return hipGetLastError();
    }
    const int pw = attn_decode_pairs_per_wg(a, B, H);
    with_beam_rows(a.beams, [&](auto kb) {
        constexpr int KB = decltype(kb)::value;
        auto packed = [&](auto pwc) {
            constexpr int PW = decltype(pwc)::value;
            hipLaunchKernelGGL((attn_decode_mfma_kernel<KB, 3, PW, 1>), dim3((p.n_pairs + PW - 1) / PW), dim3(64 * PW), 0, s, p);
        };
        if (pw == 8) { if constexpr (KB < 8) packed(std::integral_constant<int, 8>{}); }
        else if (pw == 4) packed(std::integral_constant<int, 4>{});
        else if (pw == 2) packed(std::integral_constant<int, 2>{});
        else packed(std::integral_constant<int, 1>{});
    });
    return hipGetLastError();
}

}
```

generativeimage2text_amd/csrc/kernels_search.hip:

```cpp
#include "gitmi_common.h"
#include "launchers.h"
#include "ban_rules.h"

namespace gitmi {

template <int NT>
__device__ __forceinline__ void ban_fill_ngram(const BanRow& br, const int* hist, int t, int* tbl) {
    for (int i = threadIdx.x; i < HIST_SLOTS; i += NT) tbl[i] = -1;
    __syncthreads();
    for (int i = threadIdx.x; i <= ban_ngram_last(br, t); i += NT)
        if (ban_ngram_hit(br, hist, t, i)) hist_insert(tbl, hist[i + br.n - 1]);
    __syncthreads();
}
__device__ __forceinline__ bool ban_test(const BanRow& br, const int* tbl, int c) {
    return ban_static(br, c) || (br.n > 0 && hist_contains(tbl, c));
}

template <int MMAX, int NT, bool BAN = false>
__global__ __launch_bounds__(NT) void row_topm_kernel(const float* __restrict__ logits, int ldl, int V,
                                                       const int* __restrict__ ids, int ld_ids, int cur_len,
                                                       const int* __restrict__ plen, int beams, int suppress_kind,
                                                       float rep_penalty, float* __restrict__ part_val,
                                                       int* __restrict__ part_idx, float2* __restrict__ part_lse, BanArgs ban) {
    constexpr int NW = NT / 64;
    __shared__ int s_hist[HIST_SLOTS];
    __shared__ float s_val[NT * MMAX];
    __shared__ int s_idx[NT * MMAX];
    __shared__ float s_red[2 * NW];
    __shared__ int s_redi[2 * NW];
    __shared__ int s_owner;

    const int r = blockIdx.x, tid = threadIdx.x, lane = tid & 63, wave = tid >> 6;
    const float* x = logits + (size_t)r * ldl;
    const bool suppress = suppress_kind && cur_len > plen[r / beams];
    const int last = suppress ? ids[(size_t)r * ld_ids + cur_len - 1] : -1;
    float* cv = part_val + (size_t)r * MMAX;
    int* ci = part_idx + (size_t)r * MMAX;
    const bool pen = ids != nullptr && rep_penalty != 0.f && rep_penalty != 1.f;
    if (pen) {
        for (int i = tid; i < HIST_SLOTS; i += NT) s_hist[i] = -1;
        __syncthreads();
        for (int s = tid; s < cur_len; s += NT) hist_insert(s_hist, ids[(size_t)r * ld_ids + s]);
        __syncthreads();
    }

    BanRow br{};
    int* s_ban = nullptr;
    if constexpr (BAN) {
        __shared__ int s_ban_tbl[HIST_SLOTS];
        s_ban = s_ban_tbl;
        br = ban_row(ban, r / beams, plen[r / beams], cur_len);
        ban_fill_ngram<NT>(br, ids + (size_t)r * ld_ids, cur_len, s_ban);
    }

    float tv[MMAX];
    int ti[MMAX];
#pragma unroll
    for (int j = 0; j < MMAX; ++j) { tv[j] = -INFINITY; ti[j] = 0x7fffffff; }
    float mx = -INFINITY, sm = 0.f;
    auto feed = [&](float v, int i) {
        if constexpr (BAN) { if (ban_test(br, s_ban, i)) v = -10000.f; }
        if (pen && hist_contains(s_hist, i)) v = rep_penalize(v, rep_penalty);
        if (i == last) v = -10000.f;
        if (v > mx) { sm = sm * __expf(mx - v) + 1.f; mx = v; }
        else if (mx != -INFINITY) sm += __expf(v - mx);
        if (v > tv[MMAX - 1]) {
            tv[MMAX - 1] = v; ti[MMAX - 1] = i;
#pragma unroll
            for (int j = MMAX - 1; j > 0; --j) {
                if (tv[j] > tv[j - 1]) {
                    const float a = tv[j]; tv[j] = tv[j - 1]; tv[j - 1] = a;
                    const int c = ti[j]; ti[j] = ti[j - 1]; ti[j - 1] = c;
                }
            }
        }
    };
    if ((ldl & 3) == 0 && (reinterpret_cast<uintptr_t>(logits) & 15) == 0) {
        const int nchunk = V >> 2;
        const f32x4_t* x4 = reinterpret_cast<const f32x4_t*>(x);
        int c = tid;
        for (; c + 3 * NT < nchunk; c += 4 * NT) {
            f32x4_t q[4];
#pragma unroll
            for (int u = 0; u < 4; ++u) q[u] = x4[c + u * NT];
#pragma unroll
// ... 261 lines not shown
    __shared__ int s_j[TRIE_NT / 64];
    const int b = blockIdx.x, tid = threadIdx.x, lane = tid & 63, wave = tid >> 6;
    constexpr int NW = TRIE_NT / 64;
    const int P = plen[b];
    if (cur_len < P) return;
    const bool first = cur_len == P;
    const int last = ids[(size_t)b * ld_ids + cur_len - 1];
    if (!first && last == eos) {
        if (tid == 0) { part_val[b] = 0.f; part_idx[b] = eos; part_lse[b] = float2{0.f, 1.f}; }
        return;
    }
    const float* x = logits + (size_t)b * ldl;
    const int sup = first ? -1 : last;
    float mx = -INFINITY, mn = INFINITY;
    int am = 0x7fffffff;
    for (int i = tid; i < V; i += TRIE_NT) {
        const float v = i == sup ? -10000.f : x[i];
        if (v > mx) { mx = v; am = i; }
        mn = fminf(mn, v);
    }
#pragma unroll
    for (int o = 32; o > 0; o >>= 1) {
        const float ov = __shfl_xor(mx, o, 64);
        const int oi = __shfl_xor(am, o, 64);
        if (ov > mx || (ov == mx && oi < am)) { mx = ov; am = oi; }
        mn = fminf(mn, __shfl_xor(mn, o, 64));
    }
    if (lane == 0) { s_f[wave] = mx; s_i[wave] = am; s_g[wave] = mn; }
    __syncthreads();
    mx = s_f[0]; am = s_i[0]; mn = s_g[0];
#pragma unroll
    for (int w = 1; w < NW; ++w) {
        if (s_f[w] > mx || (s_f[w] == mx && s_i[w] < am)) { mx = s_f[w]; am = s_i[w]; }
        mn = fminf(mn, s_g[w]);
    }
    __syncthreads();
    float sm = 0.f;
    for (int i = tid; i < V; i += TRIE_NT) sm += __expf((i == sup ? -10000.f : x[i]) - mx);
    sm = wave_sum(sm);
    if (lane == 0) s_f[wave] = sm;
    __syncthreads();
    float tot = 0.f;
#pragma unroll
    for (int w = 0; w < NW; ++w) tot += s_f[w];
    __syncthreads();
    const float logsum = logf(tot);
    const float bonus = (mx - mn) + 1.0f;
    const int node = tr.cursor[b];
    const int e0 = node >= 0 ? tr.child_off[node] : 0, e1 = node >= 0 ? tr.child_off[node + 1] : 0;
    float bv = -INFINITY;
    int bt = 0x7fffffff, be = -1;
    for (int e = e0 + tid; e < e1; e += TRIE_NT) {
        const int t = tr.child_tok[e];
        if (t < 0 || t >= V) continue;
        const float xv = t == sup ? -10000.f : x[t];
        const float v = ((xv - mx) - logsum) + bonus;
        if (v > bv || (v == bv && t < bt)) { bv = v; bt = t; be = e; }
    }
#pragma unroll
    for (int o = 32; o > 0; o >>= 1) {
        const float ov = __shfl_xor(bv, o, 64);
        const int ot = __shfl_xor(bt, o, 64), oe = __shfl_xor(be, o, 64);
        if (ov > bv || (ov == bv && ot < bt)) { bv = ov; bt = ot; be = oe; }
    }
    if (lane == 0) { s_f[wave] = bv; s_i[wave] = bt; s_j[wave] = be; }
    __syncthreads();
    if (tid == 0) {
        bv = s_f[0]; bt = s_i[0]; be = s_j[0];
        for (int w = 1; w < NW; ++w)
            if (s_f[w] > bv || (s_f[w] == bv && s_i[w] < bt)) { bv = s_f[w]; bt = s_i[w]; be = s_j[w]; }
        const float plain = (mx - mx) - logsum;
        const bool take_valid = be >= 0 && (bv > plain || (bv == plain && bt <= am));
        part_val[b] = take_valid ? bv : plain;
        part_idx[b] = take_valid ? bt : am;
        part_lse[b] = float2{0.f, 1.f};
        tr.cursor[b] = take_valid ? tr.child_node[be] : -1;
    }
}

__device__ __forceinline__ double length_norm(int len, double alpha) {
    return pow(5.0 + (double)len, alpha) / pow(6.0, alpha);
}

constexpr int SS_KMAX = 8;
constexpr int SS_CMAX = 16;

__device__ __forceinline__ int ids_at(const SearchState& st, int buf, int r, int s) { return st.ids[buf][(size_t)r * st.T + s]; }

template <typename TOut, int SLOTS>
__global__ __launch_bounds__(256) void search_step_kernel(SearchState st, int src, int cur_len, StepCands in,
                                                          EmbedArgs em) {
    __shared__ float c_val[SS_KMAX][SS_CMAX];
    __shared__ int c_idx[SS_KMAX][SS_CMAX];
    __shared__ int sel_src[SS_KMAX], sel_word[SS_KMAX];
    __shared__ float sel_score[SS_KMAX];
    __shared__ int s_nadd, s_add_slot[SS_CMAX * 2], s_add_row[SS_CMAX * 2];
    __shared__ float s_score[SS_KMAX];
    __shared__ int s_last[SS_KMAX];
    __shared__ int s_done, s_hyp_n, s_hyp_cnt, s_stop;
    __shared__ double s_hyp_worst, s_len_cur, s_len_last;
    __shared__ double s_hscore[SS_NHMAX];
    __shared__ int s_hseq[SS_NHMAX];
    __shared__ float s_part[8];

    const int tid = threadIdx.x, lane = tid & 63, wave = tid >> 6;
    const int b = blockIdx.x;
    const int k = st.k, pn = st.pn, T = st.T;
    const int dst = src ^ 1;
    const int P = st.plen[b];
    const bool forced = cur_len < P;
    const bool first = cur_len == P;
    const int M = st.kind == 0 ? (first ? k : pn) : (st.sampled ? pn : pn * k);

    if (tid == 0) s_nadd = 0;
    {
        const int t2 = tid - 64;
        if (t2 >= 0 && t2 < k) {
            s_score[t2] = st.score[src][b * k + t2];
            s_last[t2] = cur_len > 0 ? ids_at(st, src, b * k + t2, cur_len - 1) : -1;
        }
        if (t2 == 8) s_done = st.done[b];
        if (t2 == 9) s_hyp_n = st.hyp_n[b];
        if (t2 == 10) s_hyp_cnt = st.hyp_cnt[b];
        if (t2 == 11) s_stop = st.stop[b];
        if (t2 == 12) s_hyp_worst = st.hyp_worst[b];
        if (t2 == 13) s_len_cur = st.len_norm[cur_len];
        if (t2 == 14) s_len_last = st.len_norm[T - 1];
        if (t2 >= 16 && t2 < 16 + st.nh) {
            s_hscore[t2 - 16] = st.hyp_score[(size_t)b * st.nh + t2 - 16];
            s_hseq[t2 - 16] = st.hyp_seq[(size_t)b * st.nh + t2 - 16];
        }
    }

    if (!forced) {
        for (int j = wave; j < k; j += 4) {
            const int r = b * k + j;
            if (st.kind == 0 && first && j > 0) break;
            const int last = ids_at(st, src, r, cur_len - 1);
            if (st.kind == 0 && !first && last == st.eos) {
                if (lane < M) {
                    c_val[j][lane] = lane == 0 ? 0.f : -INFINITY;
                    c_idx[j][lane] = lane == 0 ? st.eos : (lane - 1 < st.eos ? lane - 1 : lane);
                }
                continue;
            }
            float hv[4][SLOTS];
            int hi[4][SLOTS];
            float pm = -INFINITY, ps = 0.f;
#pragma unroll
            for (int q = 0; q < 4; ++q) {
                const int p = lane + 64 * q;
                const bool ok = p < in.nparts;
                if (ok) {
                    const float2 ml = in.part_lse[(size_t)r * in.nparts + p];
                    if (ml.x > pm) { ps = ps * __expf(pm - ml.x) + ml.y; pm = ml.x; }
                    else if (ml.x != -INFINITY) ps += ml.y * __expf(ml.x - pm);
                }
                const size_t base = ((size_t)r * in.nparts + (ok ? p : 0)) * SLOTS;
#pragma unroll
                for (int e = 0; e < SLOTS; ++e) {
                    hv[q][e] = ok ? in.part_val[base + e] : -INFINITY;
                    hi[q][e] = ok ? in.part_idx[base + e] : 0x7fffffff;
                }
            }
            const float bm = wave_max(pm);
            const float part = wave_sum(pm == -INFINITY ? 0.f : ps * __expf(pm - bm));
            const float lse = bm + logf(part);
            for (int round = 0; round < M; ++round) {
                float v = hv[0][0];
                int id = hi[0][0], who = 0;
#pragma unroll
                for (int q = 1; q < 4; ++q)
                    if (hv[q][0] > v || (hv[q][0] == v && hi[q][0] < id)) { v = hv[q][0]; id = hi[q][0]; who = q; }
                int own = lane;
#pragma unroll
                for (int o = 32; o > 0; o >>= 1) {
                    const float ov = __shfl_xor(v, o, 64);
                    const int oi = __shfl_xor(id, o, 64);
                    const int ow = __shfl_xor(own, o, 64);
                    if (ov > v || (ov == v && oi < id)) { v = ov; id = oi; own = ow; }
                }
                if (lane == 0) {
                    c_val[j][round] = v - lse;
                    c_idx[j][round] = id == 0x7fffffff ? 0 : id;
                }
                if (own == lane) {
#pragma unroll
                    for (int q = 0; q < 4; ++q)
                        if (q == who) {
#pragma unroll
                            for (int e = 0; e + 1 < SLOTS; ++e) { hv[q][e] = hv[q][e + 1]; hi[q][e] = hi[q][e + 1]; }
                            hv[q][SLOTS - 1] = -INFINITY; hi[q][SLOTS - 1] = 0x7fffffff;
                        }
                }
            }
        }
    }
    __syncthreads();

    if (tid == 0) {
        if (forced) {
            const int word = (int)st.start[(size_t)b * st.ld_start + cur_len];
            for (int j = 0; j < k; ++j) { sel_src[j] = b * k + j; sel_word[j] = word; sel_score[j] = st.score[src][b * k + j]; }
        } else if (st.kind == 0) {
            if (!first && s_stop == 0) {
                int all_eos = 1;
                for (int j = 0; j < k; ++j)
                    if (s_last[j] != st.eos) all_eos = 0;
                if (all_eos) { st.stop[b] = cur_len; atomicAdd(&st.info[0], 1); }
            }
            if (first) {
                for (int j = 0; j < k; ++j) {
                    sel_src[j] = b * k; sel_word[j] = c_idx[0][j]; sel_score[j] = c_val[0][j];
                }
                if (k == 1) st.early[b] = c_idx[0][0] == st.eos ? 1 : 0;
            } else {
                unsigned long long used = 0ull;
                for (int j = 0; j < k; ++j) {
                    float best = 0.f; int bc = -1;
                    for (int c = 0; c < k * pn; ++c) {
                        if (used >> c & 1ull) continue;
                        const float v = c_val[c / pn][c % pn] + s_score[c / pn];
                        if (bc < 0 || v > best) { best = v; bc = c; }
                    }
                    used |= 1ull << bc;
                    sel_src[j] = b * k + bc / pn; sel_word[j] = c_idx[bc / pn][bc % pn]; sel_score[j] = best;
                }
            }
        } else {
            const int V = st.V;
            const int ncand = pn * k;
            int headp[SS_KMAX];
            for (int j = 0; j < k; ++j) headp[j] = 0;
            float n_score[SS_CMAX * 2]; int n_beam[SS_CMAX * 2], n_word[SS_CMAX * 2];
            float n_max = -INFINITY;
            for (int c = 0; c < ncand; ++c) {
                if (st.sampled) {
                    const int j = c / pn, d = c % pn;
                    n_score[c] = c_val[j][d] + s_score[j]; n_beam[c] = c % k; n_word[c] = c_idx[j][d];
                } else {
                    float best = 0.f; int bj = -1; long long bflat = 0;
                    for (int j = 0; j < k; ++j) {
                        if (headp[j] >= M) continue;
                        const float v = c_val[j][headp[j]] + s_score[j];
                        const long long flat = (long long)j * V + c_idx[j][headp[j]];
                        if (bj < 0 || v > best || (v == best && flat < bflat)) { best = v; bj = j; bflat = flat; }
                    }
                    n_score[c] = best; n_beam[c] = bj; n_word[c] = c_idx[bj][headp[bj]];
                    headp[bj]++;
                }
                n_max = fmaxf(n_max, n_score[c]);
            }
            const int nh = st.nh;
            double* h_score = st.hyp_score + (size_t)b * nh;
            int* h_len = st.hyp_len + (size_t)b * nh;
            int* h_seq = st.hyp_seq + (size_t)b * nh;
            const int was_done = s_done;
            int is_done = was_done;
            int hyp_n = s_hyp_n, hyp_cnt = s_hyp_cnt;
            double hyp_worst = s_hyp_worst;
            if (!is_done && hyp_n >= nh) {
                is_done = hyp_worst >= (double)n_max / s_len_last;
            }
            if (is_done && !was_done) { atomicAdd(&st.info[0], 1); st.done[b] = is_done; }
            int nb = 0;
            if (!is_done) {
                for (int c = 0; c < ncand && nb < k; ++c) {
                    const int word = n_word[c];
                    if (word == st.eos || cur_len + 1 == T) {
                        const double sc = (double)n_score[c] / s_len_cur;
                        const int n = hyp_n;
                        if (n < nh || sc > hyp_worst) {
                            int slot = n;
                            if (n < nh) {
                                hyp_n = n + 1;
                                hyp_worst = sc < hyp_worst ? sc : hyp_worst;
                            } else {
                                slot = 0;
                                for (int i = 1; i < nh; ++i)
                                    if (s_hscore[i] < s_hscore[slot] || (s_hscore[i] == s_hscore[slot] && s_hseq[i] < s_hseq[slot])) slot = i;
                                double w = sc;
                                for (int i = 0; i < nh; ++i)
                                    if (i != slot && s_hscore[i] < w) w = s_hscore[i];
                                hyp_worst = w;
                            }
                            s_hscore[slot] = sc; s_hseq[slot] = hyp_cnt;
                            h_score[slot] = sc;
                            h_len[slot] = cur_len;
                            h_seq[slot] = hyp_cnt++;
                            s_add_slot[s_nadd] = slot; s_add_row[s_nadd] = b * k + n_beam[c];
                            ++s_nadd;
                        }
                    } else {
                        sel_score[nb] = n_score[c]; sel_word[nb] = word; sel_src[nb] = b * k + n_beam[c];
                        ++nb;
                    }
                }
                if (hyp_n != s_hyp_n) st.hyp_n[b] = hyp_n;
                if (hyp_cnt != s_hyp_cnt) st.hyp_cnt[b] = hyp_cnt;
                if (hyp_worst != s_hyp_worst) st.hyp_worst[b] = hyp_worst;
            }
            if (nb < k) {
                const int pad_row = st.prefixed ? b * k : 0;
                for (int j = 0; j < k; ++j) { sel_score[j] = 0.f; sel_word[j] = st.eos; sel_src[j] = pad_row; }
            }
        }
        if (b == 0) st.info[2] += 1;
    }
    __syncthreads();

    for (int a = 0; a < s_nadd; ++a) {
        int* ht = st.hyp_tok + ((size_t)b * st.nh + s_add_slot[a]) * T;
        for (int s = tid; s < cur_len; s += 256) ht[s] = ids_at(st, src, s_add_row[a], s);
    }
    for (int idx = tid; idx < k * cur_len; idx += 256) {
        const int j = idx / cur_len, s = idx - j * cur_len;
        const int r = b * k + j, rs = sel_src[j];
        st.ids[dst][(size_t)r * T + s] = st.ids[src][(size_t)rs * T + s];
        st.kv_src[dst][(size_t)r * T + s] = st.kv_src[src][(size_t)rs * T + s];
    }
    if (tid < k) {
        const int r = b * k + tid;
        st.ids[dst][(size_t)r * T + cur_len] = sel_word[tid];
        st.kv_src[dst][(size_t)r * T + cur_len] = r;
        st.score[dst][r] = sel_score[tid];
    }

    if (em.words == nullptr || cur_len + 1 >= T) return;
    const int D = em.D;
    if (k == 1) {
        const int r = b;
        int tok = sel_word[0];
        tok = tok < 0 ? 0 : (tok >= em.vocab ? em.vocab - 1 : tok);
        const int c = tid * 4;
        const bool on = c < D;
        f32x4_t a = {0.f, 0.f, 0.f, 0.f}, g4 = a, b4 = a;
        if (on) {
            const f32x4_t w4 = *reinterpret_cast<const f32x4_t*>(em.words + (size_t)tok * D + c);
            const f32x4_t p4 = *reinterpret_cast<const f32x4_t*>(em.positions + (size_t)cur_len * D + c);
            g4 = *reinterpret_cast<const f32x4_t*>(em.gamma + c);
            b4 = *reinterpret_cast<const f32x4_t*>(em.beta + c);
#pragma unroll
            for (int q = 0; q < 4; ++q) a[q] = w4[q] + p4[q];
        }
        const float sum = wave_sum(a[0] + a[1] + a[2] + a[3]);
        if (lane == 0) s_part[wave] = sum;
        __syncthreads();
        const float mean = (s_part[0] + s_part[1] + s_part[2] + s_part[3]) / (float)D;
        float q2 = 0.f;
        if (on) {
#pragma unroll
            for (int q = 0; q < 4; ++q) { const float d = a[q] - mean; q2 += d * d; }
        }
        q2 = wave_sum(q2);
        if (lane == 0) s_part[4 + wave] = q2;
        __syncthreads();
        const float rstd = rsqrtf((s_part[4] + s_part[5] + s_part[6] + s_part[7]) / (float)D + em.eps);
        if (on) {
            float o[4];
#pragma unroll
            for (int q = 0; q < 4; ++q) o[q] = (a[q] - mean) * rstd * g4[q] + b4[q];
            *reinterpret_cast<f32x4_t*>(em.h_f + (size_t)r * D + c) = f32x4_t{o[0], o[1], o[2], o[3]};
            TOut* ht = reinterpret_cast<TOut*>(em.h_t);
            if constexpr (sizeof(TOut) == 4) {
                *reinterpret_cast<f32x4_t*>(ht + (size_t)r * D + c) = f32x4_t{o[0], o[1], o[2], o[3]};
            } else {
                uint2 t;
                t.x = pack2bf(o[0], o[1]);
                t.y = pack2bf(o[2], o[3]);
                const size_t off = em.frag ? frag_offset(r, c, D >> 5) : (size_t)r * D + c;
                *reinterpret_cast<uint2*>(ht + off) = t;
            }
        }
        return;
    }
    for (int j = wave; j < k; j += 4) {
        const int r = b * k + j;
        int tok = sel_word[j];
        tok = tok < 0 ? 0 : (tok >= em.vocab ? em.vocab - 1 : tok);
        f32x4_t a[4], g4[4], b4[4];
#pragma unroll
        for (int i = 0; i < 4; ++i) {
            const int c = (lane + 64 * i) * 4;
            a[i] = g4[i] = b4[i] = f32x4_t{0.f, 0.f, 0.f, 0.f};
            if (c < D) {
                const f32x4_t w4 = *reinterpret_cast<const f32x4_t*>(em.words + (size_t)tok * D + c);
                const f32x4_t p4 = *reinterpret_cast<const f32x4_t*>(em.positions + (size_t)cur_len * D + c);
                g4[i] = *reinterpret_cast<const f32x4_t*>(em.gamma + c);
                b4[i] = *reinterpret_cast<const f32x4_t*>(em.beta + c);
#pragma unroll
                for (int q = 0; q < 4; ++q) a[i][q] = w4[q] + p4[q];
            }
        }
        float part[4];
#pragma unroll
        for (int i = 0; i < 4; ++i) part[i] = wave_sum(a[i][0] + a[i][1] + a[i][2] + a[i][3]);
        const float mean = (part[0] + part[1] + part[2] + part[3]) / (float)D;
#pragma unroll
        for (int i = 0; i < 4; ++i) {
            float q2 = 0.f;
            if ((lane + 64 * i) * 4 < D) {
#pragma unroll
                for (int q = 0; q < 4; ++q) { const float d = a[i][q] - mean; q2 += d * d; }
            }
            part[i] = wave_sum(q2);
        }
        const float rstd = rsqrtf((part[0] + part[1] + part[2] + part[3]) / (float)D + em.eps);
#pragma unroll
        for (int i = 0; i < 4; ++i) {
            const int c = (lane + 64 * i) * 4;
            if (c < D) {
                float o[4];
#pragma unroll
                for (int q = 0; q < 4; ++q) o[q] = (a[i][q] - mean) * rstd * g4[i][q] + b4[i][q];
                *reinterpret_cast<f32x4_t*>(em.h_f + (size_t)r * D + c) = f32x4_t{o[0], o[1], o[2], o[3]};
                TOut* ht = reinterpret_cast<TOut*>(em.h_t);
                if constexpr (sizeof(TOut) == 4) {
                    *reinterpret_cast<f32x4_t*>(ht + (size_t)r * D + c) = f32x4_t{o[0], o[1], o[2], o[3]};
                } else {
                    uint2 t;
                    t.x = pack2bf(o[0], o[1]);
                    t.y = pack2bf(o[2], o[3]);
                    const size_t off = em.frag ? frag_offset(r, c, D >> 5) : (size_t)r * D + c;
                    *reinterpret_cast<uint2*>(ht + off) = t;
                }
            }
        }
    }
}

__global__ void search_init_kernel(SearchState st) {
    const int R = st.B * st.k;
    for (int i = blockIdx.x * blockDim.x + threadIdx.x; i < R * st.T; i += gridDim.x * blockDim.x) {
        const int r = i / st.T, s = i % st.T;
        const int b = r / st.k;
        st.ids[0][i] = s < st.plen[b] ? (int)st.start[(size_t)b * st.ld_start + s] : st.eos;
        st.kv_src[0][i] = r;
    }
    if (blockIdx.x == 0) {
        for (int r = threadIdx.x; r < R; r += blockDim.x) {
            st.score[0][r] = (st.kind == 1 && r % st.k > 0) ? -1e9f : 0.f;
        }
        for (int b = threadIdx.x; b < st.B; b += blockDim.x) {
            st.done[b] = 0; st.hyp_n[b] = 0; st.hyp_cnt[b] = 0; st.hyp_worst[b] = 1e9; st.stop[b] = 0; st.early[b] = 0;
        }
        if (threadIdx.x < 4) st.info[threadIdx.x] = 0;
        for (int len = threadIdx.x; len <= st.T; len += blockDim.x) st.len_norm[len] = length_norm(len, st.length_penalty);
    }
}

__global__ void search_finish_kernel(SearchState st, int cur, int cur_len, long long* __restrict__ tokens_out,
                                     float* __restrict__ logprob_out, int* __restrict__ info_out,
                                     int* __restrict__ sent_out) {
    __shared__ int s_max_stop, s_all_stop, s_all_early;
    if (threadIdx.x == 0) { s_max_stop = 0; s_all_stop = 1; s_all_early = 1; }
    __syncthreads();
    for (int b = threadIdx.x; b < st.B; b += blockDim.x) {
        const int nout = st.kind == 0 ? 1 : st.nh;
        long long* out = tokens_out + (size_t)b * nout * st.T;
        int L = st.T, early = 0;
        if (st.kind == 0) {
            const int r = b * st.k;
            const int stop = st.stop[b];
            L = stop > 0 ? stop : cur_len;
            early = st.k == 1 ? st.early[b] : 0;
            int non_eos = 0, any_eos = 0;
            for (int s = 0; s < st.T; ++s) {
                const int tok = s < L ? st.ids[cur][(size_t)r * st.T + s] : st.eos;
                out[s] = tok;
                if (s < L) { if (tok != st.eos) ++non_eos; else any_eos = 1; }
            }
            int nv = non_eos + any_eos - st.plen[b];
            nv = nv < 1 ? 1 : nv;
            logprob_out[b] = st.score[cur][r] / (float)nv;
            if (sent_out) sent_out[2 * b + 1] = early;
            if (stop > 0) atomicMax(&s_max_stop, stop); else s_all_stop = 0;
            if (!early) s_all_early = 0;
        } else {
            const int nh = st.nh, have = st.hyp_n[b];
            const double* h_score = st.hyp_score + (size_t)b * nh;
            const int* h_seq = st.hyp_seq + (size_t)b * nh;
            unsigned taken = 0u;
            for (int i = 0; i < nh; ++i) {
                int best = -1;
                for (int j = 0; j < have; ++j) {
                    if ((taken >> j) & 1u) continue;
                    if (best < 0 || h_score[j] > h_score[best] || (h_score[j] == h_score[best] && h_seq[j] < h_seq[best])) best = j;
                }
                const int n = best >= 0 ? st.hyp_len[(size_t)b * nh + best] : 0;
                const int* ht = st.hyp_tok + ((size_t)b * nh + (best >= 0 ? best : 0)) * st.T;
                for (int s = 0; s < st.T; ++s) out[(size_t)i * st.T + s] = s < n ? ht[s] : st.eos;
                logprob_out[(size_t)b * nh + i] = best >= 0 ? (float)h_score[best] : -1e5f;
                if (best >= 0) taken |= 1u << best;
            }
            if (sent_out) sent_out[2 * b + 1] = 0;
        }
        if (sent_out) sent_out[2 * b] = L;
    }
    __syncthreads();
    if (threadIdx.x == 0) {
        info_out[0] = st.kind == 0 ? (s_all_stop ? s_max_stop : cur_len) : st.T;
        info_out[1] = (st.kind == 0 && st.k == 1) ? s_all_early : 0;
        info_out[2] = st.info[2];
        const int nout = st.kind == 0 ? 1 : st.nh;
        int bad = 0;
        for (int i = 0; i < st.B * nout; ++i) bad += !isfinite(logprob_out[i]);
        info_out[3] = bad;
    }
}

__global__ void search_rows_kernel(SearchState st, int cur, int cur_len, long long* __restrict__ out) {
// ... 132 lines not shown
```

generativeimage2text_amd/csrc/launchers.h:

```cpp
#pragma once
#include <hip/hip_runtime.h>
#include <stddef.h>

namespace gitmi {

struct GemmArgs {
    const void* A; const void* W; const float* bias; const float* res; void* C;
    int M, N, K;
    int lda, ldc, ldr;
    int act;
    int tiles_n, nwg;
    int ng;
    int dbg;
    int out_f16;
    int shared;
    const float2* ln_part; int ln_nparts; const float* ln_colsum; float ln_inv_d, ln_eps;
    float2* part_out;
    const float2* res_part; int res_nparts; const float* res_gamma; const float* res_beta; float res_inv_d, res_eps;
};
bool gemm_uses_p8(const GemmArgs& g, bool in_f32, bool out_f32);
hipError_t launch_gemm(const GemmArgs& g, bool in_f32, bool out_f32, hipStream_t s);
hipError_t launch_gemm_p8(GemmArgs g, bool out_f32, hipStream_t s);
bool gemm_p8_supports(const GemmArgs& g);
int gemm_p8_cost(const GemmArgs& g, int bm);
// ... 122 lines not shown
    const FeaturePiece* pieces; int pieces_n;
    const int* count;
    int stride, D;
    int* ntok; int4* meta;
};
hipError_t launch_feature_install(const FeatureArgs& a, int B, bool src16, bool dst16, hipStream_t s);

struct AttnFullArgs {
    const void* q; const void* k; const void* v; void* out;
    int ldq, ldk, ldv, ldo;
    int N, H;
    float scale;
    const int* ntok;
};
hipError_t launch_attn_full(const AttnFullArgs& a, int B, bool is_f32, int impl, hipStream_t s);

struct AttnDecodeArgs {
    const void* qkv; const void* img_k; const void* img_v; void* txt_k; void* txt_v; void* out;
    const int* kv_src;
    const int* img_of;
    int ld_src;
    int d;
    int N_img, T_max, pos, beams;
    int N_pad;
    int out_frag;
    float scale;
    int dbg;
    int pairs_per_wg;
    int stream_wgs;
    int waves_per_pair;
    int n_pairs;
    const int* ntok;
    const unsigned short* x; const unsigned short* w; const float* bias; const float* colsum;
    const float2* stats_in; int strips_in; float inv_d, eps_in;
    int M;
};
hipError_t launch_kv_repack(const void* qkv, void* kh, void* vh, int B, int N, int H, int d, hipStream_t s);
hipError_t launch_attn_decode(const AttnDecodeArgs& a, int B, int H, hipStream_t s);
hipError_t launch_kv_repack_frag(const void* qkv, void* kf, void* vt, int B, int N, int N_pad, int H, int d, hipStream_t s);
hipError_t launch_attn_decode_mfma(const AttnDecodeArgs& a, int B, int H, hipStream_t s);
int attn_decode_pairs_per_wg(const AttnDecodeArgs& a, int B, int H);
bool attn_decode_qkv_form(const AttnDecodeArgs& a, int B, int H);
inline void attn_decode_set_qkv(AttnDecodeArgs& a, const DGemmArgs& g) {
    a.x = g.A; a.w = g.W; a.bias = g.bias; a.colsum = g.colsum;
    a.stats_in = g.stats_in; a.strips_in = g.strips_in; a.inv_d = g.inv_d; a.eps_in = g.eps_in; a.M = g.M;
}
hipError_t launch_attn_decode_qkv(const AttnDecodeArgs& a, int B, int H, hipStream_t s);

constexpr int SS_NHMAX = 8;
struct SearchState {
    int B, k, pn, T, V, eos, kind;
    int prefixed;
    int sampled;
    double length_penalty;
    double* len_norm;
    const long long* start;
    int ld_start;
    const int* plen;
    int* ids[2];
    int* kv_src[2];
    float* score[2];
    int* done;
    int nh;
    int* hyp_n;
    int* hyp_cnt;
    double* hyp_worst;
    double* hyp_score;
    int* hyp_len;
    int* hyp_seq;
    int* hyp_tok;
    int* stop;
    int* early;
    int* info;
};
struct StepCands {
    const float* part_val; const int* part_idx; const float2* part_lse;
    int nparts, slots;
};
struct EmbedArgs {
    const float* words; const float* positions; const float* gamma; const float* beta; float eps;
    float* h_f; void* h_t; int D, vocab;
    int frag;
};
int row_topm_slots(int M);
hipError_t launch_sample_rows(const float* logits, int ldl, int V, int R, float temperature, int top_k, float top_p,
                              int ndraw, unsigned long long seed, int step, float* part_val, int* part_idx,
                              float2* part_lse, float* filtered_out, const int* ids, int ld_ids, int cur_len,
                              float rep_penalty, int stride, hipStream_t s,
                              const BanArgs* ban = nullptr, const int* plen = nullptr, int beams = 1);
struct TrieArgs {
    const int* child_off; const int* child_tok; const int* child_node;
    int* cursor;
};
hipError_t launch_trie_select(const float* logits, int ldl, int V, const int* ids, int ld_ids, int cur_len, const int* plen,
                              int eos, const TrieArgs& tr, int B, float* part_val, int* part_idx, float2* part_lse,
                              hipStream_t s);
hipError_t launch_row_topm(const float* logits, int ldl, int V, const int* ids, int ld_ids, int cur_len,
                           const int* plen, int beams, int suppress_kind, float rep_penalty, int M, int R,
                           float* part_val, int* part_idx, float2* part_lse, hipStream_t s, const BanArgs* ban = nullptr);
hipError_t launch_search_step(const SearchState& st, int src, int cur_len, const StepCands& in, const EmbedArgs& em,
                              bool t_is_f32, hipStream_t s);
hipError_t launch_search_init(const SearchState& st, hipStream_t s);
hipError_t launch_search_finish(const SearchState& st, int cur, int cur_len, long long* tokens_out,
                                float* logprob_out, int* info_out, int* sent_out, hipStream_t s);
hipError_t launch_search_rows(const SearchState& st, int cur, int cur_len, long long* out, hipStream_t s);
hipError_t launch_fill_start(long long* start, int ld, const long long* prefix, int ldp, int shared, int sos, int B, int P,
                             hipStream_t s);
hipError_t launch_load_ids(const long long* tokens, int R, int t, int* ids, int* kv_src, int ld, hipStream_t s);

struct TreeNodes {
    int* tok;
    int* depth;
    int* parent;
    int* end;
};
hipError_t launch_score_embed_ln(const long long* tokens, int ld, int Q, int Lp, const float* words, const float* positions,
                                 const float* gamma, const float* beta, float eps, float* h_f, void* h_t, bool t_is_f32,
                                 int D, int vocab, int max_pos, hipStream_t s, const TreeNodes* tree = nullptr);
hipError_t launch_score_attn(const void* qkv, const void* img_kv, const int* image_of, void* out, int Q, int H, int d,
                             int N_img, int Lp, float scale, bool is_f32, hipStream_t s, const int* ntok = nullptr,
                             float2* stats = nullptr, const int* node_end = nullptr);
hipError_t launch_score_attn_map(const void* qkv, const void* img_kv, const int* image_of, const int* ntok, const float2* stats,
                                 const int* lens, float* out, size_t out_sq, size_t out_sj, int Tc, int Q, int H, int N_img,
                                 int Lp, float scale, bool is_f32, int* bad, hipStream_t s);
int score_head_tiles(int V);
hipError_t launch_score_head(const void* A, int lda, const void* W, const float* bias, const int* tgt, int M, int V, int K,
                             float4* part, float* zt, hipStream_t s);
hipError_t launch_score_rowstats(const float* logits, int ldl, int V, const int* tgt, int row_off, int rows, float4* part,
                                 float* zt, hipStream_t s);
hipError_t launch_score_targets(const long long* tokens, int ld, int Lp, const int* lens, int V, int M, int* tgt,
                                hipStream_t s);
hipError_t launch_score_combine(const float4* part, int ntiles, const float* zt, const int* tgt, int M, int Lp, int ld, int V,
                                float2* out, int* bad, hipStream_t s);
hipError_t launch_score_info(const int* bad, int Q, int ld, int* info, hipStream_t s, int i1 = 0, int i2 = 0);
hipError_t launch_tree_structure(const long long* packed, int ld, int Q, int Lp, const int* lens, int V, int max_depth,
                                 const TreeNodes& nd, int* bad, hipStream_t s);
hipError_t launch_tree_gather_dot(const void* A, int lda, const void* W, const float* bias, const TreeNodes& nd, int Lp, int M,
                                  int K, float* zt, hipStream_t s);
hipError_t launch_tree_gather_logits(const float* logits, int ldl, int row_off, int rows, const TreeNodes& nd, int Lp, int M,
                                     float* zt, hipStream_t s);
hipError_t launch_tree_combine(const float4* part, int ntiles, const float* zt, const TreeNodes& nd, int M, int Lp, int ld, int V,
                               float2* out, int* bad, hipStream_t s);

hipError_t launch_preprocess(const unsigned char* rgb, int H, int W, int crop, unsigned char* tmp, float* out, hipStream_t s);
hipError_t launch_preprocess_batch(const unsigned char* rgb, const long long* desc, int n, int crop, unsigned char* tmp, float* out,
                                   hipStream_t s);
size_t preprocess_batch_workspace(const long long* desc, int n, int crop);
hipError_t launch_resize_crop_norm(const uint8_t* rgb, int H, int W, int nh, int nw, int top, int left, int ch, int cw,
                                   uint8_t* tmp, float* out, hipStream_t s);

}
```

Measured before the change: 11620 captions/s.

## Fuse greedy search step into layer-0 decode attention and im2col directly from frames

Two changes. The per-step search/select/embed kernel is folded into the first decoder layer's fused QKV+attention kernel, so each wave computes candidate selection, the token append and the embedding layernorm inline, then feeds the result straight into the QKV input. This removes one kernel launch and a round trip through global memory per decode step. Separately, the device-to-device copy of input frames into staging buffers is dropped, and im2col now runs directly from the caller's frames before the encoder graph replays. The trade-off is extra shared memory and register pressure in the attention kernel, plus im2col moving outside the captured graph.

```diff
diff --git a/generativeimage2text_amd/csrc/engine.hip b/generativeimage2text_amd/csrc/engine.hip
--- a/generativeimage2text_amd/csrc/engine.hip
+++ b/generativeimage2text_amd/csrc/engine.hip
@@ -330,8 +330,16 @@
     return st;
 }
 
+static int im2col_frames(gitmi_engine* e, const float* const* frames, int F_eff, int B, hipStream_t s) {
+    const int g2 = e->N - 1;
+    for (int fr = 0; fr < F_eff; ++fr)
+        HIPCK(launch_im2col(frames[fr], (char*)e->patches + (size_t)fr * B * g2 * e->Kp_pad * e->pol.esz, e->pol.f32, B,
+                            e->H, e->W, e->cfg.patch, e->Kp, e->Kp_pad, s));
+    return 0;
+}
+
 static int encode_frames_impl(gitmi_engine* e, const float* const* frames, int F, int B, float* feats_out,
-                              hipStream_t s, int stride = 0) {
+                              hipStream_t s, int stride = 0, bool patches_ready = false) {
     const gitmi_config& c = e->cfg;
     const int D = c.vit_width, N = e->N;
     const int F_eff = c.num_frames > 0 ? std::min(F, c.num_frames) : F;
@@ -344,10 +352,8 @@
     const size_t slot = (size_t)3 * e->max_pixels;
     if (e->ragged)
         HIPCK(launch_im2col_ragged(e->frame_stage[0], slot, e->rg_meta, e->patches, e->pol.f32, B, N, c.patch, e->Kp, e->Kp_pad, s));
-    else
-    for (int fr = 0; fr < F_eff; ++fr)
-        HIPCK(launch_im2col(frames[fr], (char*)e->patches + (size_t)fr * B * g2 * e->Kp_pad * e->pol.esz, e->pol.f32, B,
-                            e->H, e->W, c.patch, e->Kp, e->Kp_pad, s));
+    else if (!patches_ready)
+        RCK(im2col_frames(e, frames, F_eff, B, s));
     RCK(gemm(e, s, e->patches, e->Kp_pad, e->w.conv_w, nullptr, nullptr, 0, e->patch_out, D, true, BI * g2, D, e->Kp_pad, 0,
              TAG_GEMM_VIT));
     Stream x = vit_stream(e, M);
@@ -444,40 +450,64 @@
     return dgemm_ln(A, f.w, f.bias, f.colsum, ln, C, c_frag, act, M, N, K);
 }
 
-static int decode_layers_impl(gitmi_engine* e, const int* kv_src, int ld_ids, int pos, int R, int beams, hipStream_t s) {
+static DLn decode_ln_prev(const gitmi_engine* e, int l) {
+    const int d = e->cfg.dec_hidden;
+    const DecLayerW* Lp = l > 0 ? &e->w.dec[l - 1] : nullptr;
+    return DLn{e->stats_o, d / 16, 1.0f / (float)d, 1e-12f, Lp ? Lp->lnog : nullptr, Lp ? Lp->lnob : nullptr};
+}
+static AttnDecodeArgs decode_attn_args(gitmi_engine* e, int l, const int* kv_src, int ld_ids, int pos, int R, int beams,
+                                       DGemmArgs* g, bool* qkv_inside) {
+    const gitmi_config& c = e->cfg;
+    const int d = c.dec_hidden;
+    const int B = R / beams;
+    const bool chain = e->pol.skinny && !e->pol.f32;
+    AttnDecodeArgs a{};
+    a.qkv = e->d_qkv; a.img_k = e->img_kh[l]; a.img_v = e->img_vh[l]; a.txt_k = e->txt_k[l]; a.txt_v = e->txt_v[l]; a.out = e->d_ctx;
+    a.kv_src = kv_src; a.ld_src = ld_ids; a.d = d; a.N_img = e->cur_Nimg; a.T_max = c.max_text_len;
+    a.img_of = e->img_identity ? nullptr : e->img_of_dev;
+    a.pos = pos; a.beams = beams; a.scale = 0.125f;
+    a.out_frag = chain ? 1 : 0;
+    a.N_pad = round_up(e->cur_Nimg, 32);
+    a.dbg = e->pol.attn_dbg;
+    a.waves_per_pair = e->pol.attn_nh;
+    a.pairs_per_wg = e->pol.attn_pw > 0 ? e->pol.attn_pw : e->pol.shared_device ? 8 : 4;
+    const bool stream_ok = !e->pol.shared_device && a.N_pad <= 8 * 32 && B * c.dec_heads >= 384 && e->pol.attn_nh != 2;
+    a.stream_wgs = e->pol.attn_stream >= 0 ? e->pol.attn_stream : stream_ok ? 192 : 0;
+    if (e->keyed) { a.ntok = e->rg_ntok; a.stream_wgs = 0; }
+    *qkv_inside = false;
+    if (chain) {
+        const DLn ln_prev = decode_ln_prev(e, l);
+        *g = dgemm_ln(l == 0 ? e->d_ht : e->xo_b, e->w.dec[l].qkv_f, l > 0 ? &ln_prev : nullptr, e->d_qkv, 0, 0, R, 3 * d, d);
+        attn_decode_set_qkv(a, *g);
+        *qkv_inside = !GITMI_SKIPPED(e, ~0) && !e->pol.dgemm_dbg && attn_decode_qkv_form(a, B, c.dec_heads) && attn_decode_pairs_per_wg(a, B, c.dec_heads) == 8;
+    }
+    return a;
+}
+
+static int decode_layers_impl(gitmi_engine* e, const int* kv_src, int ld_ids, int pos, int R, int beams, hipStream_t s,
+                              const SearchFuseArgs* fuse = nullptr) {
     const gitmi_config& c = e->cfg;
     const int d = c.dec_hidden, ffn = c.dec_ffn;
     const int B = R / beams;
     const bool chain = e->pol.skinny && !e->pol.f32;
     for (int l = 0; l < c.dec_layers; ++l) {
         const DecLayerW& L = e->w.dec[l];
-        const DecLayerW* Lp = l > 0 ? &e->w.dec[l - 1] : nullptr;
-        const DLn ln_prev{e->stats_o, d / 16, 1.0f / (float)d, 1e-12f, Lp ? Lp->lnog : nullptr, Lp ? Lp->lnob : nullptr};
+        const DLn ln_prev = decode_ln_prev(e, l);
         const DLn ln_a{e->stats_a, d / 16, 1.0f / (float)d, 1e-12f, L.lnag, L.lnab};
-        const DLn* ln_o = Lp ? &ln_prev : nullptr;
-        AttnDecodeArgs a{};
-        a.qkv = e->d_qkv; a.img_k = e->img_kh[l]; a.img_v = e->img_vh[l]; a.txt_k = e->txt_k[l]; a.txt_v = e->txt_v[l]; a.out = e->d_ctx;
-        a.kv_src = kv_src; a.ld_src = ld_ids; a.d = d; a.N_img = e->cur_Nimg; a.T_max = c.max_text_len;
-        a.img_of = e->img_identity ? nullptr : e->img_of_dev;
-        a.pos = pos; a.beams = beams; a.scale = 0.125f;
-        a.out_frag = chain ? 1 : 0;
-        a.N_pad = round_up(e->cur_Nimg, 32);
-        a.dbg = e->pol.attn_dbg;
-        a.waves_per_pair = e->pol.attn_nh;
-        a.pairs_per_wg = e->pol.attn_pw > 0 ? e->pol.attn_pw : e->pol.shared_device ? 8 : 4;
-        const bool stream_ok = !e->pol.shared_device && a.N_pad <= 8 * 32 && B * c.dec_heads >= 384 && e->pol.attn_nh != 2;
-        a.stream_wgs = e->pol.attn_stream >= 0 ? e->pol.attn_stream : stream_ok ? 192 : 0;
-        if (e->keyed) { a.ntok = e->rg_ntok; a.stream_wgs = 0; }
+        const DLn* ln_o = l > 0 ? &ln_prev : nullptr;
+        DGemmArgs g{};
         bool qkv_inside = false;
+        const AttnDecodeArgs a = decode_attn_args(e, l, kv_src, ld_ids, pos, R, beams, &g, &qkv_inside);
         if (chain) {
-            const DGemmArgs g = dgemm_ln(l == 0 ? e->d_ht : e->xo_b, L.qkv_f, ln_o, e->d_qkv, 0, 0, R, 3 * d, d);
-            attn_decode_set_qkv(a, g);
-            qkv_inside = !GITMI_SKIPPED(e, ~0) && !e->pol.dgemm_dbg && attn_decode_qkv_form(a, B, c.dec_heads) && attn_decode_pairs_per_wg(a, B, c.dec_heads) == 8;
             if (!qkv_inside && !GITMI_SKIPPED(e, 2) && !GITMI_SKIPPED(e, 16)) RCK(dgemm(e, s, g));
         } else {
             RCK(gemm(e, s, e->d_ht, d, L.wqkv, L.bqkv, nullptr, 0, e->d_qkv, 3 * d, e->pol.f32, R, 3 * d, d, 0, TAG_GEMM_OTHER));
         }
-        if (e->pol.f32) HIPCK(launch_attn_decode(a, B, c.dec_heads, s));
+        if (l == 0 && fuse) {
+            if (!qkv_inside) return fail("decode step: the search step was left to an attention launch that cannot run it");
+            HIPCK(launch_attn_decode_qkv_search(a, *fuse, B, c.dec_heads, s));
+        }
+        else if (e->pol.f32) HIPCK(launch_attn_decode(a, B, c.dec_heads, s));
         else if (qkv_inside) HIPCK(launch_attn_decode_qkv(a, B, c.dec_heads, s));
         else if (!GITMI_SKIPPED(e, 1)) HIPCK(launch_attn_decode_mfma(a, B, c.dec_heads, s));
         if (chain) {
@@ -713,11 +743,12 @@
     return 0;
 }
 
-static int search_step_impl(gitmi_engine* e, const StepCands& cands, bool embed, hipStream_t s) {
+static int search_step_impl(gitmi_engine* e, const StepCands& cands, bool embed, hipStream_t s, SearchFuseArgs* defer = nullptr) {
     const SearchState& st = e->ss;
     const int cur_len = e->ss_len;
     if (cur_len >= st.T) return fail("search_advance: sequence already at max_steps");
-    HIPCK(launch_search_step(st, e->ss_cur, cur_len, cands, embed_args(e, embed), e->pol.f32, s));
+    if (defer) *defer = SearchFuseArgs{st, e->ss_cur, cur_len, cands, embed_args(e, embed)};
+    else HIPCK(launch_search_step(st, e->ss_cur, cur_len, cands, embed_args(e, embed), e->pol.f32, s));
     e->ss_cur ^= 1;
     e->ss_len = cur_len + 1;
     return 0;
@@ -885,12 +916,24 @@
 }
 
 static int generate_encode(gitmi_engine* e, const Request& rq, hipStream_t s) {
-    RCK(encode_frames_impl(e, rq.frames, rq.F, rq.B, nullptr, s));
+    RCK(encode_frames_impl(e, rq.frames, rq.F, rq.B, nullptr, s, 0, rq.patches_ready));
     return prefill_impl(e, s);
 }
 static int images_ready(gitmi_engine* e, const Request& rq, hipStream_t s) {
     if (rq.frames) return generate_encode(e, rq, s);
     return e->have_prefill ? 0 : prefill_impl(e, s);
+}
+
+static bool search_inside_next(gitmi_engine* e, const Request& rq, const StepCands& cands, int R, int k, bool allow_poll) {
+    const SearchState& st = e->ss;
+    const int cur_len = e->ss_len;
+    if (allow_poll || e->ban_live || e->trie_search || e->keyed || e->ragged || st.sampled) return false;
+    if (cur_len < rq.minP || cur_len + 1 >= st.T) return false;
+    DGemmArgs g{};
+    bool qkv_inside = false;
+    const AttnDecodeArgs a = decode_attn_args(e, 0, st.kv_src[e->ss_cur ^ 1], st.T, cur_len, R, k, &g, &qkv_inside);
+    if (!qkv_inside) return false;
+    return attn_decode_search_form(a, SearchFuseArgs{st, e->ss_cur, cur_len, cands, embed_args(e, true)}, R / k, e->cfg.dec_heads);
 }
 
 static int generate_decode(gitmi_engine* e, const Request& rq, hipStream_t s, bool allow_poll) {
@@ -906,13 +949,16 @@
         RCK(embed_position(e, st.ids[0], T, 0, R, s));
         e->ss_len = 1;
         StepCands cands{e->part_val, e->part_idx, e->part_lse, 1, 1};
+        SearchFuseArgs fuse{};
+        bool fused = false;
         while (e->ss_len < T) {
             const int cur_len = e->ss_len;
             SpanGuard step(e, s, TAG_STEP, 0);
-            RCK(decode_layers_impl(e, st.kv_src[e->ss_cur], T, cur_len - 1, R, k, s));
+            RCK(decode_layers_impl(e, st.kv_src[e->ss_cur], T, cur_len - 1, R, k, s, fused ? &fuse : nullptr));
             if (cur_len >= minP)
                 RCK(decode_head_impl(e, st.ids[e->ss_cur], T, cur_len, R, k, suppress, M, nullptr, 0, s, &cands));
-            RCK(search_step_impl(e, cands, true, s));
+            fused = search_inside_next(e, rq, cands, R, k, allow_poll);
+            RCK(search_step_impl(e, cands, true, s, fused ? &fuse : nullptr));
             if (allow_poll && e->ss_len > maxP && (e->ss_len - maxP) % 8 == 0 && e->ss_len < T) {
                 int h[4];
                 HIPCK(hipMemcpyAsync(h, st.info, sizeof(h), hipMemcpyDeviceToHost, s));
@@ -945,15 +991,15 @@
             sp.do_sample, sp.top_k, keep_best(sp), sp.top_p, sp.temperature, sp.repetition_penalty, sp.seed, e->ban_live ? 1 : 0};
 }
 
-static int replay(gitmi_engine* e, const Request& rq, hipStream_t x, const CapturedGraph* enc, const CapturedGraph* dec) {
+static int replay(gitmi_engine* e, const Request& rq, int F_eff, hipStream_t x, const CapturedGraph* enc, const CapturedGraph* dec) {
     const bool timed = e->profile_mode == 2;
     if (timed) {
         for (auto& ev : e->gev)
             if (!ev) HIPCK(hipEventCreate(&ev));
         HIPCK(hipEventRecord(e->gev[enc ? 0 : 1], x));
-    } else if (enc && e->enc_after && e->enc_after->enc_done) {
-        HIPCK(hipStreamWaitEvent(x, e->enc_after->enc_done, 0));
-    }
+    }
+    if (enc && !e->ragged) RCK(im2col_frames(e, rq.frames, F_eff, rq.B, x));
+    if (!timed && enc && e->enc_after && e->enc_after->enc_done) HIPCK(hipStreamWaitEvent(x, e->enc_after->enc_done, 0));
     if (enc) {
         HIPCK(enc->launch(x));
         if (timed) HIPCK(hipEventRecord(e->gev[1], x));
@@ -978,13 +1024,9 @@
         HIPCK(hipEventRecord(e->fence_in, s));
         HIPCK(hipStreamWaitEvent(x, e->fence_in, 0));
     }
-    const size_t frame_bytes = (size_t)rq.B * 3 * e->H * e->W * sizeof(float);
     const int F_eff = resident ? e->cur_F : c.num_frames > 0 ? std::min(rq.F, c.num_frames) : rq.F;
-    if (!e->ragged && !resident)
-    for (int f = 0; f < F_eff; ++f)
-        HIPCK(hipMemcpyAsync(e->frame_stage[f], rq.frames[f], frame_bytes, hipMemcpyDeviceToDevice, x));
     Request own = rq;
-    if (!resident) { own.frames = e->frame_stage.data(); own.F = F_eff; }
+    if (!resident) { own.frames = &e->frame_stage[0]; own.F = F_eff; own.patches_ready = !e->ragged; }
     own.tokens = e->out_tokens; own.logprob = e->out_lp; own.info = e->out_info; own.sent = e->out_sent;
     const GraphKey key = graph_key_of(e, rq, F_eff);
     const CapturedGraph *enc = nullptr, *dec = nullptr;
@@ -1015,7 +1057,7 @@
         enc = &e->graph_full;
         if (split) dec = &e->graph_decode;
     }
-    RCK(replay(e, rq, x, enc, dec));
+    RCK(replay(e, rq, F_eff, x, enc, dec));
     const size_t nout = (size_t)rq.Q * (size_t)keep_best(*rq.sp);
     HIPCK(hipMemcpyAsync(rq.tokens, e->out_tokens, nout * rq.sp->max_steps * sizeof(long long), hipMemcpyDefault, x));
     HIPCK(hipMemcpyAsync(rq.logprob, e->out_lp, nout * sizeof(float), hipMemcpyDefault, x));
diff --git a/generativeimage2text_amd/csrc/engine_state.h b/generativeimage2text_amd/csrc/engine_state.h
--- a/generativeimage2text_amd/csrc/engine_state.h
+++ b/generativeimage2text_amd/csrc/engine_state.h
@@ -74,6 +74,7 @@
     const gitmi_search* sp;
     long long* tokens; float* logprob; int32_t* info;
     int32_t* sent;
+    bool patches_ready = false;
 };
 
 struct ModelWeights {
diff --git a/generativeimage2text_amd/csrc/engine_weights.hip b/generativeimage2text_amd/csrc/engine_weights.hip
--- a/generativeimage2text_amd/csrc/engine_weights.hip
+++ b/generativeimage2text_amd/csrc/engine_weights.hip
@@ -209,9 +209,8 @@
     HIPCK(hipStreamCreateWithFlags(&e->own_stream, hipStreamNonBlocking));
     HIPCK(hipEventCreateWithFlags(&e->fence_in, hipEventDisableTiming));
     HIPCK(hipEventCreateWithFlags(&e->fence_out, hipEventDisableTiming));
-    e->frame_stage.resize(c.max_frames);
-    for (int f = 0; f < c.max_frames; ++f)
-        RCK(dev_alloc_t(e, &e->frame_stage[f], (size_t)c.max_batch * 3 * e->max_pixels));
+    e->frame_stage.resize(1);
+    RCK(dev_alloc_t(e, &e->frame_stage[0], (size_t)c.max_batch * 3 * e->max_pixels));
     RCK(dev_alloc_t(e, &e->rg_meta, (size_t)c.max_batch));
     RCK(dev_alloc_t(e, &e->rg_ntok, (size_t)c.max_batch));
     return 0;
diff --git a/generativeimage2text_amd/csrc/kernels_attn_decode.hip b/generativeimage2text_amd/csrc/kernels_attn_decode.hip
--- a/generativeimage2text_amd/csrc/kernels_attn_decode.hip
+++ b/generativeimage2text_amd/csrc/kernels_attn_decode.hip
@@ -1,6 +1,7 @@
 #include "gitmi_common.h"
 #include "launchers.h"
 #include "dgemm_shared.h"
+#include "search_step_dev.h"
 #include <algorithm>
 #include <type_traits>
 
@@ -409,8 +410,37 @@
     asm volatile("" ::: "memory");
 }
 
-template <int TI>
-__global__ __launch_bounds__(64 * AQ_PW) void attn_decode_qkv_kernel(AttnDecodeArgs a) {
+__device__ __forceinline__ void search_wave_sync() {
+    asm volatile("s_waitcnt lgkmcnt(0)" ::: "memory");
+    __builtin_amdgcn_wave_barrier();
+}
+template <typename Sink>
+__device__ __forceinline__ void search_step_wave(const SearchFuseArgs& sf, int b, int lane, SearchShared& sh, bool write, Sink&& sink) {
+    const SearchState& st = sf.st;
+    const int src = sf.src, cur_len = sf.cur_len;
+    const int P = st.plen[b];
+    const bool forced = cur_len < P, first = cur_len == P;
+    const int M = first ? st.k : st.pn;
+    if (lane == 0) {
+        sh.s_nadd = 0;
+        sh.s_score[0] = st.score[src][b];
+        sh.s_last[0] = ids_at(st, src, b, cur_len - 1);
+        sh.s_stop = write ? st.stop[b] : 0;
+    }
+    if (!forced) search_row_candidates<1>(st, sf.in, src, cur_len, b, 0, first, M, lane, sh);
+    search_wave_sync();
+    if (lane == 0) {
+        search_select_ar(st, src, cur_len, b, forced, first, sh, write);
+        if (write && b == 0) st.info[2] += 1;
+    }
+    search_wave_sync();
+    if (write) search_append<64>(st, src, cur_len, b, sh, lane);
+    embed_ln_wave<bf16_t>(sf.em, b, sh.sel_word[0], cur_len, lane, write, sink);
+}
+
+struct NoSearchArgs {};
+template <int TI, bool SEARCH>
+__global__ __launch_bounds__(64 * AQ_PW) void attn_decode_qkv_kernel(AttnDecodeArgs a, std::conditional_t<SEARCH, SearchFuseArgs, NoSearchArgs> sf) {
     constexpr int KB = 1;
     __shared__ __attribute__((aligned(16))) f32x4_t red[AQ_STRIPS][4][1][64];
     __shared__ __attribute__((aligned(16))) bf16_t rows[AQ_PW][3 * HD];
@@ -460,7 +490,7 @@
                                 : __builtin_nontemporal_load(reinterpret_cast<const bf16x8_t*>(vp + dt * 512));
         }
     };
-    load_k(0);
+    if constexpr (!SEARCH) load_k(0);
 
     const int ksteps = a.d >> 5, N = 3 * a.d;
     const int slice = wave & 3;
@@ -468,7 +498,25 @@
     const int rt = b0 >> 4;
     auto strip_of = [&](int ls) { return (ls >> 2) * (a.d >> 4) + p.h * 4 + (ls & 3); };
     bf16x8_t xf[DW_KS][1];
-    load_x_slice(xf, reinterpret_cast<const bf16_t*>(a.x), rt, ks, ksteps, lane);
+    if constexpr (SEARCH) {
+        __shared__ __attribute__((aligned(16))) bf16_t xs[16 * 4 * DW_KS * 32];
+        __shared__ SearchShared ssh[AQ_PW];
+        const int row = (b0 & 15) + wave;
+        auto put = [&](int r16, int c, uint2 v) { *reinterpret_cast<uint2*>(&xs[frag_offset(r16, c, ksteps)]) = v; };
+        for (int c = lane * 4; c < a.d; c += 256) {
+            put(row ^ 8, c, uint2{0u, 0u});
+            if (!p.on) put(row, c, uint2{0u, 0u});
+        }
+        if (p.on)
+            search_step_wave(sf, b, lane, ssh[wave], p.h == 0, [&](int c, const float (&o)[4]) {
+                put(row, c, uint2{pack2bf(o[0], o[1]), pack2bf(o[2], o[3])});
+            });
+        load_k(0);
+        attn_lds_barrier();
+        load_x_slice(xf, xs, 0, ks, ksteps, lane);
+    } else {
+        load_x_slice(xf, reinterpret_cast<const bf16_t*>(a.x), rt, ks, ksteps, lane);
+    }
 #pragma unroll 2
     for (int u = 0; u < AQ_STRIPS / 2; ++u) {
         const int ls = (wave >> 2) * (AQ_STRIPS / 2) + u;
@@ -750,7 +798,27 @@
     AttnDecodeArgs p = a;
     p.n_pairs = B * H;
     const int total = H * ((B + AQ_PW - 1) / AQ_PW);
-    hipLaunchKernelGGL((attn_decode_qkv_kernel<3>), dim3(8 * ((total + 7) / 8)), dim3(64 * AQ_PW), 0, s, p);
+    hipLaunchKernelGGL((attn_decode_qkv_kernel<3, false>), dim3(8 * ((total + 7) / 8)), dim3(64 * AQ_PW), 0, s, p, NoSearchArgs{});
+    return hipGetLastError();
+}
+
+bool attn_decode_search_form(const AttnDecodeArgs& a, const SearchFuseArgs& sf, int B, int H) {
+    if (!attn_decode_qkv_form(a, B, H) || a.stats_in) return false;
+    const SearchState& st = sf.st;
+    if (st.kind != 0 || st.k != 1 || st.pn != 1 || st.B != B) return false;
+    if (sf.in.slots != 1 || sf.in.nparts < 1 || sf.in.nparts > 256) return false;
+    if (!sf.in.part_val || !sf.in.part_idx || !sf.in.part_lse) return false;
+    if (sf.cur_len != a.pos || sf.cur_len < 1 || sf.cur_len + 1 >= st.T || st.T > a.T_max) return false;
+    const EmbedArgs& em = sf.em;
+    return em.words && em.D == a.d && em.frag && em.h_f && em.h_t == (const void*)a.x;
+}
+
+hipError_t launch_attn_decode_qkv_search(const AttnDecodeArgs& a, const SearchFuseArgs& sf, int B, int H, hipStream_t s) {
+    if (!attn_decode_search_form(a, sf, B, H)) return hipErrorInvalidValue;
+    AttnDecodeArgs p = a;
+    p.n_pairs = B * H;
+    const int total = H * ((B + AQ_PW - 1) / AQ_PW);
+    hipLaunchKernelGGL((attn_decode_qkv_kernel<3, true>), dim3(8 * ((total + 7) / 8)), dim3(64 * AQ_PW), 0, s, p, sf);
     return hipGetLastError();
 }
 
diff --git a/generativeimage2text_amd/csrc/kernels_search.hip b/generativeimage2text_amd/csrc/kernels_search.hip
--- a/generativeimage2text_amd/csrc/kernels_search.hip
+++ b/generativeimage2text_amd/csrc/kernels_search.hip
@@ -1,6 +1,7 @@
 #include "gitmi_common.h"
 #include "launchers.h"
 #include "ban_rules.h"
+#include "search_step_dev.h"
 
 namespace gitmi {
 
@@ -428,31 +429,26 @@
     return pow(5.0 + (double)len, alpha) / pow(6.0, alpha);
 }
 
-constexpr int SS_KMAX = 8;
-constexpr int SS_CMAX = 16;
-
-__device__ __forceinline__ int ids_at(const SearchState& st, int buf, int r, int s) { return st.ids[buf][(size_t)r * st.T + s]; }
-
 template <typename TOut, int SLOTS>
 __global__ __launch_bounds__(256) void search_step_kernel(SearchState st, int src, int cur_len, StepCands in,
                                                           EmbedArgs em) {
-    __shared__ float c_val[SS_KMAX][SS_CMAX];
-    __shared__ int c_idx[SS_KMAX][SS_CMAX];
-    __shared__ int sel_src[SS_KMAX], sel_word[SS_KMAX];
-    __shared__ float sel_score[SS_KMAX];
-    __shared__ int s_nadd, s_add_slot[SS_CMAX * 2], s_add_row[SS_CMAX * 2];
-    __shared__ float s_score[SS_KMAX];
-    __shared__ int s_last[SS_KMAX];
-    __shared__ int s_done, s_hyp_n, s_hyp_cnt, s_stop;
-    __shared__ double s_hyp_worst, s_len_cur, s_len_last;
-    __shared__ double s_hscore[SS_NHMAX];
-    __shared__ int s_hseq[SS_NHMAX];
-    __shared__ float s_part[8];
+    __shared__ SearchShared sh;
+    float (&c_val)[SS_KMAX][SS_CMAX] = sh.c_val;
+    int (&c_idx)[SS_KMAX][SS_CMAX] = sh.c_idx;
+    int (&sel_src)[SS_KMAX] = sh.sel_src, (&sel_word)[SS_KMAX] = sh.sel_word;
+    float (&sel_score)[SS_KMAX] = sh.sel_score;
+    int &s_nadd = sh.s_nadd, (&s_add_slot)[SS_CMAX * 2] = sh.s_add_slot, (&s_add_row)[SS_CMAX * 2] = sh.s_add_row;
+    float (&s_score)[SS_KMAX] = sh.s_score;
+    int (&s_last)[SS_KMAX] = sh.s_last;
+    int &s_done = sh.s_done, &s_hyp_n = sh.s_hyp_n, &s_hyp_cnt = sh.s_hyp_cnt, &s_stop = sh.s_stop;
+    double &s_hyp_worst = sh.s_hyp_worst, &s_len_cur = sh.s_len_cur, &s_len_last = sh.s_len_last;
+    double (&s_hscore)[SS_NHMAX] = sh.s_hscore;
+    int (&s_hseq)[SS_NHMAX] = sh.s_hseq;
+    float (&s_part)[8] = sh.s_part;
 
     const int tid = threadIdx.x, lane = tid & 63, wave = tid >> 6;
     const int b = blockIdx.x;
     const int k = st.k, pn = st.pn, T = st.T;
-    const int dst = src ^ 1;
     const int P = st.plen[b];
     const bool forced = cur_len < P;
     const bool first = cur_len == P;
@@ -482,97 +478,14 @@
         for (int j = wave; j < k; j += 4) {
             const int r = b * k + j;
             if (st.kind == 0 && first && j > 0) break;
-            const int last = ids_at(st, src, r, cur_len - 1);
-            if (st.kind == 0 && !first && last == st.eos) {
-                if (lane < M) {
-                    c_val[j][lane] = lane == 0 ? 0.f : -INFINITY;
-                    c_idx[j][lane] = lane == 0 ? st.eos : (lane - 1 < st.eos ? lane - 1 : lane);
-                }
-                continue;
-            }
-            float hv[4][SLOTS];
-            int hi[4][SLOTS];
-            float pm = -INFINITY, ps = 0.f;
-#pragma unroll
-            for (int q = 0; q < 4; ++q) {
-                const int p = lane + 64 * q;
-                const bool ok = p < in.nparts;
-                if (ok) {
-                    const float2 ml = in.part_lse[(size_t)r * in.nparts + p];
-                    if (ml.x > pm) { ps = ps * __expf(pm - ml.x) + ml.y; pm = ml.x; }
-                    else if (ml.x != -INFINITY) ps += ml.y * __expf(ml.x - pm);
-                }
-                const size_t base = ((size_t)r * in.nparts + (ok ? p : 0)) * SLOTS;
-#pragma unroll
-                for (int e = 0; e < SLOTS; ++e) {
-                    hv[q][e] = ok ? in.part_val[base + e] : -INFINITY;
-                    hi[q][e] = ok ? in.part_idx[base + e] : 0x7fffffff;
-                }
-            }
-            const float bm = wave_max(pm);
-            const float part = wave_sum(pm == -INFINITY ? 0.f : ps * __expf(pm - bm));
-            const float lse = bm + logf(part);
-            for (int round = 0; round < M; ++round) {
-                float v = hv[0][0];
-                int id = hi[0][0], who = 0;
-#pragma unroll
-                for (int q = 1; q < 4; ++q)
-                    if (hv[q][0] > v || (hv[q][0] == v && hi[q][0] < id)) { v = hv[q][0]; id = hi[q][0]; who = q; }
-                int own = lane;
-#pragma unroll
-                for (int o = 32; o > 0; o >>= 1) {
-                    const float ov = __shfl_xor(v, o, 64);
-                    const int oi = __shfl_xor(id, o, 64);
-                    const int ow = __shfl_xor(own, o, 64);
-                    if (ov > v || (ov == v && oi < id)) { v = ov; id = oi; own = ow; }
-                }
-                if (lane == 0) {
-                    c_val[j][round] = v - lse;
-                    c_idx[j][round] = id == 0x7fffffff ? 0 : id;
-                }
-                if (own == lane) {
-#pragma unroll
-                    for (int q = 0; q < 4; ++q)
-                        if (q == who) {
-#pragma unroll
-                            for (int e = 0; e + 1 < SLOTS; ++e) { hv[q][e] = hv[q][e + 1]; hi[q][e] = hi[q][e + 1]; }
-                            hv[q][SLOTS - 1] = -INFINITY; hi[q][SLOTS - 1] = 0x7fffffff;
-                        }
-                }
-            }
+            search_row_candidates<SLOTS>(st, in, src, cur_len, r, j, first, M, lane, sh);
         }
     }
     __syncthreads();
 
     if (tid == 0) {
-        if (forced) {
-            const int word = (int)st.start[(size_t)b * st.ld_start + cur_len];
-            for (int j = 0; j < k; ++j) { sel_src[j] = b * k + j; sel_word[j] = word; sel_score[j] = st.score[src][b * k + j]; }
-        } else if (st.kind == 0) {
-            if (!first && s_stop == 0) {
-                int all_eos = 1;
-                for (int j = 0; j < k; ++j)
-                    if (s_last[j] != st.eos) all_eos = 0;
-                if (all_eos) { st.stop[b] = cur_len; atomicAdd(&st.info[0], 1); }
-            }
-            if (first) {
-                for (int j = 0; j < k; ++j) {
-                    sel_src[j] = b * k; sel_word[j] = c_idx[0][j]; sel_score[j] = c_val[0][j];
-                }
-                if (k == 1) st.early[b] = c_idx[0][0] == st.eos ? 1 : 0;
-            } else {
-                unsigned long long used = 0ull;
-                for (int j = 0; j < k; ++j) {
-                    float best = 0.f; int bc = -1;
-                    for (int c = 0; c < k * pn; ++c) {
-                        if (used >> c & 1ull) continue;
-                        const float v = c_val[c / pn][c % pn] + s_score[c / pn];
-                        if (bc < 0 || v > best) { best = v; bc = c; }
-                    }
-                    used |= 1ull << bc;
-                    sel_src[j] = b * k + bc / pn; sel_word[j] = c_idx[bc / pn][bc % pn]; sel_score[j] = best;
-                }
-            }
+        if (forced || st.kind == 0) {
+            search_select_ar(st, src, cur_len, b, forced, first, sh, true);
         } else {
             const int V = st.V;
             const int ncand = pn * k;
@@ -655,22 +568,7 @@
     }
     __syncthreads();
 
-    for (int a = 0; a < s_nadd; ++a) {
-        int* ht = st.hyp_tok + ((size_t)b * st.nh + s_add_slot[a]) * T;
-        for (int s = tid; s < cur_len; s += 256) ht[s] = ids_at(st, src, s_add_row[a], s);
-    }
-    for (int idx = tid; idx < k * cur_len; idx += 256) {
-        const int j = idx / cur_len, s = idx - j * cur_len;
-        const int r = b * k + j, rs = sel_src[j];
-        st.ids[dst][(size_t)r * T + s] = st.ids[src][(size_t)rs * T + s];
-        st.kv_src[dst][(size_t)r * T + s] = st.kv_src[src][(size_t)rs * T + s];
-    }
-    if (tid < k) {
-        const int r = b * k + tid;
-        st.ids[dst][(size_t)r * T + cur_len] = sel_word[tid];
-        st.kv_src[dst][(size_t)r * T + cur_len] = r;
-        st.score[dst][r] = sel_score[tid];
-    }
+    search_append<256>(st, src, cur_len, b, sh, tid);
 
     if (em.words == nullptr || cur_len + 1 >= T) return;
     const int D = em.D;
@@ -693,12 +591,7 @@
         if (lane == 0) s_part[wave] = sum;
         __syncthreads();
         const float mean = (s_part[0] + s_part[1] + s_part[2] + s_part[3]) / (float)D;
-        float q2 = 0.f;
-        if (on) {
-#pragma unroll
-            for (int q = 0; q < 4; ++q) { const float d = a[q] - mean; q2 += d * d; }
-        }
-        q2 = wave_sum(q2);
+        const float q2 = wave_sum(on ? sum_sq_rounded(a, mean) : 0.f);
         if (lane == 0) s_part[4 + wave] = q2;
         __syncthreads();
         const float rstd = rsqrtf((s_part[4] + s_part[5] + s_part[6] + s_part[7]) / (float)D + em.eps);
@@ -720,59 +613,8 @@
         }
         return;
     }
-    for (int j = wave; j < k; j += 4) {
-        const int r = b * k + j;
-        int tok = sel_word[j];
-        tok = tok < 0 ? 0 : (tok >= em.vocab ? em.vocab - 1 : tok);
-        f32x4_t a[4], g4[4], b4[4];
-#pragma unroll
-        for (int i = 0; i < 4; ++i) {
-            const int c = (lane + 64 * i) * 4;
-            a[i] = g4[i] = b4[i] = f32x4_t{0.f, 0.f, 0.f, 0.f};
-            if (c < D) {
-                const f32x4_t w4 = *reinterpret_cast<const f32x4_t*>(em.words + (size_t)tok * D + c);
-                const f32x4_t p4 = *reinterpret_cast<const f32x4_t*>(em.positions + (size_t)cur_len * D + c);
-                g4[i] = *reinterpret_cast<const f32x4_t*>(em.gamma + c);
-                b4[i] = *reinterpret_cast<const f32x4_t*>(em.beta + c);
-#pragma unroll
-                for (int q = 0; q < 4; ++q) a[i][q] = w4[q] + p4[q];
-            }
-        }
-        float part[4];
-#pragma unroll
-        for (int i = 0; i < 4; ++i) part[i] = wave_sum(a[i][0] + a[i][1] + a[i][2] + a[i][3]);
-        const float mean = (part[0] + part[1] + part[2] + part[3]) / (float)D;
-#pragma unroll
-        for (int i = 0; i < 4; ++i) {
-            float q2 = 0.f;
-            if ((lane + 64 * i) * 4 < D) {
-#pragma unroll
-                for (int q = 0; q < 4; ++q) { const float d = a[i][q] - mean; q2 += d * d; }
-            }
-            part[i] = wave_sum(q2);
-        }
-        const float rstd = rsqrtf((part[0] + part[1] + part[2] + part[3]) / (float)D + em.eps);
-#pragma unroll
-        for (int i = 0; i < 4; ++i) {
-            const int c = (lane + 64 * i) * 4;
-            if (c < D) {
-                float o[4];
-#pragma unroll
-                for (int q = 0; q < 4; ++q) o[q] = (a[i][q] - mean) * rstd * g4[i][q] + b4[i][q];
-                *reinterpret_cast<f32x4_t*>(em.h_f + (size_t)r * D + c) = f32x4_t{o[0], o[1], o[2], o[3]};
-                TOut* ht = reinterpret_cast<TOut*>(em.h_t);
-                if constexpr (sizeof(TOut) == 4) {
-                    *reinterpret_cast<f32x4_t*>(ht + (size_t)r * D + c) = f32x4_t{o[0], o[1], o[2], o[3]};
-                } else {
-                    uint2 t;
-                    t.x = pack2bf(o[0], o[1]);
-                    t.y = pack2bf(o[2], o[3]);
-                    const size_t off = em.frag ? frag_offset(r, c, D >> 5) : (size_t)r * D + c;
-                    *reinterpret_cast<uint2*>(ht + off) = t;
-                }
-            }
-        }
-    }
+    for (int j = wave; j < k; j += 4)
+        embed_ln_wave<TOut>(em, b * k + j, sel_word[j], cur_len, lane, true, [](int, const float (&)[4]) {});
 }
 
 __global__ void search_init_kernel(SearchState st) {
diff --git a/generativeimage2text_amd/csrc/launchers.h b/generativeimage2text_amd/csrc/launchers.h
--- a/generativeimage2text_amd/csrc/launchers.h
+++ b/generativeimage2text_amd/csrc/launchers.h
@@ -228,6 +228,15 @@
     float* h_f; void* h_t; int D, vocab;
     int frag;
 };
+struct SearchFuseArgs {
+    SearchState st;
+    int src, cur_len;
+    StepCands in;
+    EmbedArgs em;
+};
+bool attn_decode_search_form(const AttnDecodeArgs& a, const SearchFuseArgs& sf, int B, int H);
+hipError_t launch_attn_decode_qkv_search(const AttnDecodeArgs& a, const SearchFuseArgs& sf, int B, int H, hipStream_t s);
+
 int row_topm_slots(int M);
 hipError_t launch_sample_rows(const float* logits, int ldl, int V, int R, float temperature, int top_k, float top_p,
                               int ndraw, unsigned long long seed, int step, float* part_val, int* part_idx,
diff --git a/generativeimage2text_amd/csrc/search_step_dev.h b/generativeimage2text_amd/csrc/search_step_dev.h
--- /dev/null
+++ b/generativeimage2text_amd/csrc/search_step_dev.h
@@ -0,0 +1,209 @@
+#pragma once
+#include "gitmi_common.h"
+#include "launchers.h"
+
+namespace gitmi {
+
+constexpr int SS_KMAX = 8;
+constexpr int SS_CMAX = 16;
+
+__device__ __forceinline__ int ids_at(const SearchState& st, int buf, int r, int s) { return st.ids[buf][(size_t)r * st.T + s]; }
+
+struct SearchShared {
+    float c_val[SS_KMAX][SS_CMAX];
+    int c_idx[SS_KMAX][SS_CMAX];
+    int sel_src[SS_KMAX], sel_word[SS_KMAX];
+    float sel_score[SS_KMAX];
+    int s_nadd, s_add_slot[SS_CMAX * 2], s_add_row[SS_CMAX * 2];
+    float s_score[SS_KMAX];
+    int s_last[SS_KMAX];
+    int s_done, s_hyp_n, s_hyp_cnt, s_stop;
+    double s_hyp_worst, s_len_cur, s_len_last;
+    double s_hscore[SS_NHMAX];
+    int s_hseq[SS_NHMAX];
+    float s_part[8];
+};
+
+template <int SLOTS>
+__device__ __forceinline__ void search_row_candidates(const SearchState& st, const StepCands& in, int src, int cur_len, int r, int j,
+                                                      bool first, int M, int lane, SearchShared& sh) {
+    const int last = ids_at(st, src, r, cur_len - 1);
+    if (st.kind == 0 && !first && last == st.eos) {
+        if (lane < M) {
+            sh.c_val[j][lane] = lane == 0 ? 0.f : -INFINITY;
+            sh.c_idx[j][lane] = lane == 0 ? st.eos : (lane - 1 < st.eos ? lane - 1 : lane);
+        }
+        return;
+    }
+    float hv[4][SLOTS];
+    int hi[4][SLOTS];
+    float pm = -INFINITY, ps = 0.f;
+#pragma unroll
+    for (int q = 0; q < 4; ++q) {
+        const int p = lane + 64 * q;
+        const bool ok = p < in.nparts;
+        if (ok) {
+            const float2 ml = in.part_lse[(size_t)r * in.nparts + p];
+            if (ml.x > pm) { ps = ps * __expf(pm - ml.x) + ml.y; pm = ml.x; }
+            else if (ml.x != -INFINITY) ps += ml.y * __expf(ml.x - pm);
+        }
+        const size_t base = ((size_t)r * in.nparts + (ok ? p : 0)) * SLOTS;
+#pragma unroll
+        for (int e = 0; e < SLOTS; ++e) {
+            hv[q][e] = ok ? in.part_val[base + e] : -INFINITY;
+            hi[q][e] = ok ? in.part_idx[base + e] : 0x7fffffff;
+        }
+    }
+    const float bm = wave_max(pm);
+    const float part = wave_sum(pm == -INFINITY ? 0.f : ps * __expf(pm - bm));
+    const float lse = bm + logf(part);
+    for (int round = 0; round < M; ++round) {
+        float v = hv[0][0];
+        int id = hi[0][0], who = 0;
+#pragma unroll
+        for (int q = 1; q < 4; ++q)
+            if (hv[q][0] > v || (hv[q][0] == v && hi[q][0] < id)) { v = hv[q][0]; id = hi[q][0]; who = q; }
+        int own = lane;
+#pragma unroll
+        for (int o = 32; o > 0; o >>= 1) {
+            const float ov = __shfl_xor(v, o, 64);
+            const int oi = __shfl_xor(id, o, 64);
+            const int ow = __shfl_xor(own, o, 64);
+            if (ov > v || (ov == v && oi < id)) { v = ov; id = oi; own = ow; }
+        }
+        if (lane == 0) {
+            sh.c_val[j][round] = v - lse;
+            sh.c_idx[j][round] = id == 0x7fffffff ? 0 : id;
+        }
+        if (own == lane) {
+#pragma unroll
+            for (int q = 0; q < 4; ++q)
+                if (q == who) {
+#pragma unroll
+                    for (int e = 0; e + 1 < SLOTS; ++e) { hv[q][e] = hv[q][e + 1]; hi[q][e] = hi[q][e + 1]; }
+                    hv[q][SLOTS - 1] = -INFINITY; hi[q][SLOTS - 1] = 0x7fffffff;
+                }
+        }
+    }
+}
+
+__device__ __forceinline__ void search_select_ar(const SearchState& st, int src, int cur_len, int b, bool forced, bool first,
+                                                 SearchShared& sh, bool write) {
+    const int k = st.k, pn = st.pn;
+    if (forced) {
+        const int word = (int)st.start[(size_t)b * st.ld_start + cur_len];
+        for (int j = 0; j < k; ++j) { sh.sel_src[j] = b * k + j; sh.sel_word[j] = word; sh.sel_score[j] = st.score[src][b * k + j]; }
+        return;
+    }
+    if (!first && sh.s_stop == 0) {
+        int all_eos = 1;
+        for (int j = 0; j < k; ++j)
+            if (sh.s_last[j] != st.eos) all_eos = 0;
+        if (all_eos && write) { st.stop[b] = cur_len; atomicAdd(&st.info[0], 1); }
+    }
+    if (first) {
+        for (int j = 0; j < k; ++j) {
+            sh.sel_src[j] = b * k; sh.sel_word[j] = sh.c_idx[0][j]; sh.sel_score[j] = sh.c_val[0][j];
+        }
+        if (k == 1 && write) st.early[b] = sh.c_idx[0][0] == st.eos ? 1 : 0;
+    } else {
+        unsigned long long used = 0ull;
+        for (int j = 0; j < k; ++j) {
+            float best = 0.f; int bc = -1;
+            for (int c = 0; c < k * pn; ++c) {
+                if (used >> c & 1ull) continue;
+                const float v = sh.c_val[c / pn][c % pn] + sh.s_score[c / pn];
+                if (bc < 0 || v > best) { best = v; bc = c; }
+            }
+            used |= 1ull << bc;
+            sh.sel_src[j] = b * k + bc / pn; sh.sel_word[j] = sh.c_idx[bc / pn][bc % pn]; sh.sel_score[j] = best;
+        }
+    }
+}
+
+template <int NT>
+__device__ __forceinline__ void search_append(const SearchState& st, int src, int cur_len, int b, const SearchShared& sh, int tid) {
+    const int k = st.k, T = st.T, dst = src ^ 1;
+    for (int a = 0; a < sh.s_nadd; ++a) {
+        int* ht = st.hyp_tok + ((size_t)b * st.nh + sh.s_add_slot[a]) * T;
+        for (int s = tid; s < cur_len; s += NT) ht[s] = ids_at(st, src, sh.s_add_row[a], s);
+    }
+    for (int idx = tid; idx < k * cur_len; idx += NT) {
+        const int j = idx / cur_len, s = idx - j * cur_len;
+        const int r = b * k + j, rs = sh.sel_src[j];
+        st.ids[dst][(size_t)r * T + s] = st.ids[src][(size_t)rs * T + s];
+        st.kv_src[dst][(size_t)r * T + s] = st.kv_src[src][(size_t)rs * T + s];
+    }
+    if (tid < k) {
+        const int r = b * k + tid;
+        st.ids[dst][(size_t)r * T + cur_len] = sh.sel_word[tid];
+        st.kv_src[dst][(size_t)r * T + cur_len] = r;
+        st.score[dst][r] = sh.sel_score[tid];
+    }
+}
+
+__device__ __forceinline__ float sum_sq_rounded(const f32x4_t& a, float mean) {
+#pragma clang fp contract(off)
+    float q2 = 0.f;
+#pragma unroll
+    for (int q = 0; q < 4; ++q) { const float d = a[q] - mean; q2 += d * d; }
+    return q2;
+}
+
+template <typename TOut, typename Sink>
+__device__ __forceinline__ void embed_ln_wave(const EmbedArgs& em, int r, int tok, int cur_len, int lane, bool write, Sink&& sink) {
+    const int D = em.D;
+    tok = tok < 0 ? 0 : (tok >= em.vocab ? em.vocab - 1 : tok);
+    f32x4_t a[4], g4[4], b4[4];
+#pragma unroll
+    for (int i = 0; i < 4; ++i) {
+        const int c = (lane + 64 * i) * 4;
+        a[i] = g4[i] = b4[i] = f32x4_t{0.f, 0.f, 0.f, 0.f};
+        if (c < D) {
+            const f32x4_t w4 = *reinterpret_cast<const f32x4_t*>(em.words + (size_t)tok * D + c);
+            const f32x4_t p4 = *reinterpret_cast<const f32x4_t*>(em.positions + (size_t)cur_len * D + c);
+            g4[i] = *reinterpret_cast<const f32x4_t*>(em.gamma + c);
+            b4[i] = *reinterpret_cast<const f32x4_t*>(em.beta + c);
+#pragma unroll
+            for (int q = 0; q < 4; ++q) a[i][q] = w4[q] + p4[q];
+        }
+    }
+    float part[4];
+#pragma unroll
+    for (int i = 0; i < 4; ++i) part[i] = wave_sum(a[i][0] + a[i][1] + a[i][2] + a[i][3]);
+    const float mean = (part[0] + part[1] + part[2] + part[3]) / (float)D;
+#pragma unroll
+    for (int i = 0; i < 4; ++i) {
+        float q2 = 0.f;
+        if ((lane + 64 * i) * 4 < D) {
+            q2 = sum_sq_rounded(a[i], mean);
+        }
+        part[i] = wave_sum(q2);
+    }
+    const float rstd = rsqrtf((part[0] + part[1] + part[2] + part[3]) / (float)D + em.eps);
+#pragma unroll
+    for (int i = 0; i < 4; ++i) {
+        const int c = (lane + 64 * i) * 4;
+        if (c < D) {
+            float o[4];
+#pragma unroll
+            for (int q = 0; q < 4; ++q) o[q] = (a[i][q] - mean) * rstd * g4[i][q] + b4[i][q];
+            if (write) {
+                *reinterpret_cast<f32x4_t*>(em.h_f + (size_t)r * D + c) = f32x4_t{o[0], o[1], o[2], o[3]};
+                TOut* ht = reinterpret_cast<TOut*>(em.h_t);
+                if constexpr (sizeof(TOut) == 4) {
+                    *reinterpret_cast<f32x4_t*>(ht + (size_t)r * D + c) = f32x4_t{o[0], o[1], o[2], o[3]};
+                } else {
+                    uint2 t;
+                    t.x = pack2bf(o[0], o[1]);
+                    t.y = pack2bf(o[2], o[3]);
+                    const size_t off = em.frag ? frag_offset(r, c, D >> 5) : (size_t)r * D + c;
+                    *reinterpret_cast<uint2*>(ht + off) = t;
+                }
+            }
+            sink(c, o);
+        }
+    }
+}
+
+}
```

Result: no change. 11620 captions/s (-0.1%).
